# EIDOSLAB/ProgressiveCodec

Measured on AMD Instinct MI355X. Metric: megapixels/s encode+decode (256x256 batches), higher is better.
Workload: dtype f32

## Files before the change

### include/pcodec.h

```cpp
#ifndef PCODEC_H
#define PCODEC_H

#include <stddef.h>
#include <stdint.h>

#ifdef __cplusplus
extern "C" {
#endif

#if defined(__GNUC__)
#define PC_API __attribute__((visibility("default")))
#else
#define PC_API
#endif

enum {
    PC_OK = 0,
    PC_ERR_ARG = -1,
    PC_ERR_INDEX = -2,
    PC_ERR_BUFFER = -3,
    PC_ERR_TRUNCATED = -4,
    PC_ERR_CDF = -5,
    PC_ERR_HIP = -6,
    PC_ERR_NOMEM = -7,
// ... 137 lines not shown
PC_API int pc_codec_profile_begin(pc_codec* c);
PC_API int pc_codec_profile_end(pc_codec* c, int64_t* n_launches, double* total_ms, double* total_flops);
PC_API int pc_codec_profile_bytes(const pc_codec* c, double* total_algorithmic_bytes);
PC_API int pc_profile_set_epoch(int device);
PC_API int pc_codec_profile_intervals(const pc_codec* c, double* t0_ms, double* t1_ms, double* flops, size_t cap, size_t* n);
PC_API int pc_codec_host_stats(const pc_codec* c, double* out, int n);

PC_API int pc_selftest_packed_gelu(uint64_t* n_mismatch, uint64_t* n_nan_payload);

#define PC_TEST_MAX_SEG 8
typedef struct pc_test_conv_desc {
    int nseg;
    const float* seg_ptr[PC_TEST_MAX_SEG];
    int seg_ld[PC_TEST_MAX_SEG];
    int seg_nch[PC_TEST_MAX_SEG];
    int smallc;
    int64_t in_sb, in_sy, in_sx, in_sc;
    int Cin, B, H, W;
    int kind, k, stride;
    int square;
    const float* w; const float* bias; int Cout;
    int epi;
    const float* aux0; int ld0;
    const float* aux1; int ld1;
    const float* fg_gamma; const float* fg_beta;
    float* out;
    int64_t out_sb, out_sy, out_sx, out_sc;
    int pixel_shuffle;
    float* out_relu;
    int ngroup;
    const float* g1_seg0; const float* g1_w; const float* g1_bias; float* g1_out;
    int tile_cfg;
} pc_test_conv_desc;
#define PC_PLAN_UNI_16_3 1
#define PC_PLAN_UNI_32_2 2
#define PC_PLAN_UNI_32_3 3
#define PC_PLAN_UNI_32_2_SQ 4
#define PC_PLAN_UNI_OTHER 5
#define PC_PLAN_L0_64x64 6
#define PC_PLAN_L0_64x64_SMALLC 7
#define PC_PLAN_L0_128x32 8
#define PC_PLAN_L0_128x32_SMALLC 9
#define PC_PLAN_L0_128x128 10
#define PC_PLAN_L0_128x128_SMALLC 11
#define PC_PLAN_IN_GDN 12
#define PC_FORM_SLOW 1
#define PC_FORM_DIRECT 2
#define PC_FORM_TABLE 3
#define PC_FORM_NCHW_PS 4
#define PC_FORM_L0_DIRECT 5
#define PC_FORM_L0_GENERIC 6
#define PC_FORM_IN_GDN 7
PC_API int pc_test_conv(const pc_test_conv_desc* d, int* plan, void* stream);

typedef struct pc_test_stage_desc {
    int size;
    int kind;
    int B;
    int HW;
    int C;
    int H;
    int W;
    const float* scale;
    int ld_scale;
    const float* mu;
    int ld_mu;
    const float* y;
    int ld_y;
    const float* ybase;
    int ld_ybase;
    const float* yadd;
    int ld_yadd;
    const float* thr;
    int mask_mode;
    const float* mask_src;
    int64_t mask_sb;
    const float* table;
    int ntable;
    float bound;
    int32_t* sym;
    int32_t* idx;
    uint8_t* idx8;
    float* mask;
    float* yhat;
    int ld_yhat;
    float* lik;
    int64_t lik_sb;
    const float* x;
    int ld_x;
    const float* aux0;
    const float* aux1;
    float* out;
    float* out2;
    int heads;
    int ws;
    int shift;
    int bias_ji;
    float fscale;
    int inverse;
    float q;
    uint32_t* work;
    int64_t sb;
    const float* thr_bar;
    int mode_star;
    int mode_bar;
} pc_test_stage_desc;
// ... 25 lines not shown
```

### progressivecodec_amd/_lib.py

```python
import ctypes as C
import os

_HERE = os.path.dirname(os.path.abspath(__file__))
LIB_PATH = os.environ.get("PC_LIB") or os.path.join(_HERE, "libpcodec.so")

PC_OK = 0
ERRORS = {-1: "PC_ERR_ARG", -2: "PC_ERR_INDEX", -3: "PC_ERR_BUFFER", -4: "PC_ERR_TRUNCATED", -5: "PC_ERR_CDF",
          -6: "PC_ERR_HIP", -7: "PC_ERR_NOMEM", -8: "PC_ERR_STATE", -9: "PC_ERR_MISSING"}

EXPORTS = [
    "pc_version", "pc_strerror", "pc_last_hip_error", "pc_rans_bound", "pc_rans_encode_with_indexes",
    "pc_rans_decode_with_indexes", "pc_rans_encode_batch", "pc_rans_decode_batch", "pc_pmf_to_quantized_cdf",
    "pc_pack_conv_weight", "pc_conv2d_nhwc", "pc_gdn_nhwc", "pc_win_attention_nhwc", "pc_mask_quantile_threshold",
    "pc_gc_prep_encode", "pc_gc_prep_decode_index", "pc_gc_dequantize", "pc_codec_create", "pc_codec_destroy",
    "pc_codec_set_tensor", "pc_codec_set_tables", "pc_codec_finalize", "pc_codec_set_threads", "pc_codec_compress",
    "pc_codec_num_slices", "pc_codec_get_string", "pc_codec_decompress", "pc_codec_read_tap", "pc_codec_read_tap_i32",
    "pc_codec_profile_begin", "pc_codec_profile_end", "pc_codec_compress_levels", "pc_codec_get_level_string",
    "pc_codec_decompress_levels", "pc_codec_forward", "pc_codec_set_cust_map", "pc_codec_strings_size", "pc_codec_copy_strings",
    "pc_codec_decompress_packed", "pc_host_pool_plan", "pc_rans_decode_stream", "pc_codec_set_scale_table", "pc_codec_profile_bytes", "pc_contract_id", "pc_rans_decode_batch_u8", "pc_codec_set_rem",
    "pc_codec_host_stats", "pc_codec_set_rem_checkpoint", "pc_codec_set_option", "pc_selftest_packed_gelu", "pc_profile_set_epoch", "pc_codec_profile_intervals",
    "pc_codec_set_post_filter", "pc_codec_post_filter",
    "pc_codec_set_model", "pc_codec_wacnn_compress", "pc_codec_wacnn_decompress", "pc_codec_wacnn_forward",
    "pc_test_conv", "pc_codec_set_topology", "pc_test_stage",
]


class PcodecError(RuntimeError):
    def __init__(self, code, where=""):
        self.code = code
        msg = lib().pc_strerror(code).decode() if _lib is not None else ""
        hip = lib().pc_last_hip_error() if (_lib is not None and code == -6) else 0
        super().__init__(f"{where}: {ERRORS.get(code, code)} ({msg})" + (f" hipError={hip}" if hip else ""))


_lib = None


def lib():
    global _lib
    if _lib is None:
        if not os.path.exists(LIB_PATH):
            raise ImportError(
                f"{LIB_PATH} not found: build it with `python -c 'import __graft_entry__ as g; g.build()'` "
                "(hipcc --offload-arch=gfx950).  progressivecodec_amd has no CPU fallback.")
        L = C.CDLL(LIB_PATH)
        vp, i32p, f32p, u8p, sz = C.c_void_p, C.POINTER(C.c_int32), C.POINTER(C.c_float), C.POINTER(C.c_uint8), C.c_size_t
        L.pc_version.restype = C.c_char_p
        L.pc_contract_id.restype = C.c_uint32
        L.pc_strerror.restype = C.c_char_p
        L.pc_strerror.argtypes = [C.c_int]
        L.pc_rans_bound.restype = sz
        L.pc_rans_bound.argtypes = [sz]
        L.pc_rans_encode_with_indexes.argtypes = [vp, vp, sz, vp, C.c_int, C.c_int, vp, vp, vp, sz, C.POINTER(sz)]
        L.pc_rans_decode_with_indexes.argtypes = [vp, sz, vp, sz, vp, C.c_int, C.c_int, vp, vp, vp]
        L.pc_rans_decode_batch_u8.argtypes = [vp, vp, sz, vp, sz, vp, C.c_int, C.c_int, vp, vp, vp, C.c_int]
        L.pc_rans_decode_stream.argtypes = [vp, sz, vp, vp, sz, vp, C.c_int, C.c_int, vp, vp, vp]
        L.pc_host_pool_plan.argtypes = [C.POINTER(C.c_int), C.POINTER(C.c_int), C.POINTER(C.c_int)]
        L.pc_rans_encode_batch.argtypes = [vp, vp, sz, sz, vp, C.c_int, C.c_int, vp, vp, vp, sz, vp, C.c_int]
        L.pc_rans_decode_batch.argtypes = [vp, vp, sz, vp, sz, vp, C.c_int, C.c_int, vp, vp, vp, C.c_int]
        L.pc_pmf_to_quantized_cdf.argtypes = [vp, C.c_int, C.c_int, vp]
        L.pc_pack_conv_weight.argtypes = [vp, C.c_int, C.c_int, C.c_int, C.c_int, vp]
        L.pc_conv2d_nhwc.argtypes = [vp, C.c_int, C.c_int, C.c_int, C.c_int, vp, vp, C.c_int, C.c_int, C.c_int, C.c_int,
                                     C.c_int, C.c_int, vp, vp]
        L.pc_gdn_nhwc.argtypes = [vp, C.c_int, C.c_int, C.c_int, C.c_int, vp, vp, C.c_int, vp, vp]
        L.pc_win_attention_nhwc.argtypes = [vp, vp, C.c_int, C.c_int, C.c_int, C.c_int, C.c_int, C.c_int, C.c_int, vp, vp]
        L.pc_mask_quantile_threshold.argtypes = [vp, C.c_int, C.c_int, C.c_int, C.c_int, C.c_float, vp, vp]
        L.pc_gc_prep_encode.argtypes = [vp, C.c_int, vp, C.c_int, vp, C.c_int, vp, C.c_int, vp, C.c_int, C.c_int, C.c_int,
                                        vp, C.c_int, C.c_float, vp, vp, vp, vp, C.c_int, vp]
        L.pc_gc_prep_decode_index.argtypes = [vp, C.c_int, vp, C.c_int, C.c_int, C.c_int, vp, C.c_int, C.c_float, vp, vp, vp]
        L.pc_gc_dequantize.argtypes = [vp, vp, C.c_int, C.c_int, C.c_int, vp, C.c_int, vp]
        L.pc_codec_create.argtypes = [C.POINTER(vp), C.c_int]
        L.pc_codec_destroy.argtypes = [vp]
        L.pc_codec_destroy.restype = None
        L.pc_codec_set_tensor.argtypes = [vp, C.c_char_p, vp, C.c_int, C.POINTER(C.c_int64), C.c_int]
        L.pc_codec_set_tables.argtypes = [vp, C.c_int, vp, C.c_int, C.c_int, vp, vp]
        L.pc_codec_finalize.argtypes = [vp]
        L.pc_codec_set_threads.argtypes = [vp, C.c_int]
        L.pc_codec_set_option.argtypes = [vp, C.c_char_p, C.c_int]
        if hasattr(L, "pc_selftest_packed_gelu"):
            L.pc_selftest_packed_gelu.argtypes = [C.POINTER(C.c_uint64), C.POINTER(C.c_uint64)]
        if hasattr(L, "pc_test_conv"):
            L.pc_test_conv.argtypes = [vp, C.POINTER(C.c_int), vp]
        if hasattr(L, "pc_test_stage"):
            L.pc_test_stage.argtypes = [vp, C.POINTER(C.c_int), vp]
        L.pc_codec_compress.argtypes = [vp, vp, C.c_int, C.c_int, C.c_int, C.c_double, C.c_int, vp, vp]
        L.pc_codec_num_slices.argtypes = [vp]
        L.pc_codec_get_string.argtypes = [vp, C.c_int, C.c_int, C.POINTER(vp), C.POINTER(sz)]
        L.pc_codec_decompress.argtypes = [vp, vp, vp, C.c_int, vp, vp, C.c_int, C.c_int, C.c_int, C.c_double, C.c_int, vp, vp]
        L.pc_codec_compress_levels.argtypes = [vp, vp, C.c_int, C.c_int, C.c_int, vp, C.c_int, C.c_int, vp, vp]
        L.pc_codec_get_level_string.argtypes = [vp, C.c_int, C.c_int, C.c_int, C.POINTER(vp), C.POINTER(sz)]
        L.pc_codec_decompress_levels.argtypes = [vp, vp, vp, vp, vp, C.c_int, C.c_int, C.c_int, vp, C.c_int, C.c_int, vp, vp]
        L.pc_codec_set_cust_map.argtypes = [vp, vp]
        L.pc_codec_set_rem.argtypes = [vp, vp, C.c_int]
        L.pc_codec_set_rem_checkpoint.argtypes = [vp, vp]
        L.pc_codec_set_post_filter.argtypes = [vp, C.c_int]
        L.pc_codec_post_filter.argtypes = [vp, C.c_int, vp, C.c_int, C.c_int, C.c_int, vp, vp]
        L.pc_codec_set_model.argtypes = [vp, C.c_int]
        L.pc_codec_set_topology.argtypes = [vp, vp]
        L.pc_codec_wacnn_compress.argtypes = [vp, vp, C.c_int, C.c_int, C.c_int, vp]
        L.pc_codec_wacnn_decompress.argtypes = [vp, vp, sz, vp, vp, C.c_int, C.c_int, C.c_int, vp, vp]
        L.pc_codec_wacnn_forward.argtypes = [vp, vp, C.c_int, C.c_int, C.c_int, vp, vp, vp, vp]
        L.pc_codec_strings_size.argtypes = [vp, C.POINTER(sz), C.POINTER(C.c_int)]
        L.pc_codec_copy_strings.argtypes = [vp, vp, sz, vp, sz]
        L.pc_codec_decompress_packed.argtypes = [vp, vp, vp, C.c_int, C.c_int, C.c_int, vp, C.c_int, C.c_int, vp, vp]
        L.pc_codec_forward.argtypes = [vp, vp, C.c_int, C.c_int, C.c_int, C.c_double, C.c_int, vp, vp, vp, vp, C.c_int, vp]
        L.pc_codec_set_scale_table.argtypes = [vp, vp, C.c_int]
        L.pc_codec_read_tap.argtypes = [vp, C.c_char_p, vp, sz, C.POINTER(sz)]
        L.pc_codec_read_tap_i32.argtypes = [vp, C.c_char_p, vp, sz, C.POINTER(sz)]
        L.pc_codec_profile_begin.argtypes = [vp]
        L.pc_profile_set_epoch.argtypes = [C.c_int]
        L.pc_codec_profile_intervals.argtypes = [vp, vp, vp, vp, sz, C.POINTER(sz)]
        L.pc_codec_profile_bytes.argtypes = [vp, C.POINTER(C.c_double)]
        L.pc_codec_host_stats.argtypes = [vp, C.POINTER(C.c_double), C.c_int]
        L.pc_codec_profile_end.argtypes = [vp, C.POINTER(C.c_int64), C.POINTER(C.c_double), C.POINTER(C.c_double)]
        _lib = L
    return _lib


def check(code, where=""):
    if code != PC_OK:
        raise PcodecError(code, where)
```

### progressivecodec_amd/csrc/pc_codec.hip

```cpp
#include <hip/hip_runtime.h>

#include <algorithm>
#include <atomic>
#include <chrono>
#include <condition_variable>
#include <new>
#include <cmath>
#include <cstdio>
#include <cstdlib>
#include <cstring>
#include <functional>
#include <map>
#include <mutex>
#include <thread>
#include <string>
#include <vector>

#include "../../include/pcodec.h"
#include "pc_device.h"
#include "pc_host.h"

static std::atomic<int> g_last_hip{0};
struct pc_codec;
static thread_local pc_codec* g_prof = nullptr;
// ... 44 lines not shown
    bool staging_pending = false;
    pc_rowtab_cache* rowtabs = nullptr;
    std::map<std::string, HostTensor> sd;
    std::vector<void*> weight_allocs;
    std::map<std::string, DevBuf> bufs;
    struct GaW { ConvW c0, c2, c5, c7; GdnW g1, g3, g6; WamW w4, w8; };
    GaW ga[2];
    std::vector<LrrW> rem;
    int rem_levels_loaded = 0;
    int rem_n = 0;
    double rem_check[3] = {0, 0, 0};
    bool multi_enc = false;
    GsW gs[2];
    int post_mode = 0;
    UnetW unet[2];
    ConvW ha[5];
    HsW hms[2], hss[2];
    pc_topology topo{};
    ConvW joiner[NS0][3];
    Stack5W cc_mean[NS0], cc_scale[NS0], lrp[NS0], cc_mean_p[NS0], cc_scale_p[NS0], lrp_p[NS0];
    float* medians = nullptr;
    const float* cust_map = nullptr;
    const float* rem_ckpt = nullptr;
    int opt_serial = 0, opt_lanes_enc = 0, opt_lanes_dec = 0;
    int rem_mu_std = 0;
    float* eb_net = nullptr;
    float* scale_table = nullptr;
    int n_table = 0;
    float scale_bound = 0.11f;
    Tables gc, eb;
    int32_t* h_sym = nullptr; int32_t* h_idx = nullptr; size_t h_cap = 0;
    int res_slices = 0, res_B = 0;
    std::vector<char> res_level_coded;
    std::vector<hipEvent_t> lvl_events;
    hipStream_t pipe_stream = nullptr;
    std::vector<hipEvent_t> pipe_ev;
    std::vector<std::vector<uint8_t>> y_strings;
    std::vector<std::vector<uint8_t>> z_strings;
    int n_threads = 0;
    bool profile = false;
    bool profile_in_schedule = false;
    bool serial_profile() const { return profile && !profile_in_schedule; }
    std::mutex prof_mu;
    std::vector<hipEvent_t> ev;
    size_t ev_used = 0;
    double prof_flops = 0.0, prof_bytes = 0.0;
    struct ProfRec { int M, N, K, nphase, epi; double flops, bytes; double t0_ms, t1_ms; };
    std::vector<ProfRec> prof_rec;
    struct Lane { hipStream_t sA = nullptr; hipEvent_t eDone = nullptr; };
    std::vector<Lane> lanes;
    hipEvent_t eFork = nullptr;
    std::mutex buf_mu;
    double t_host_decode_ms = 0.0;
    double t_compress_ms = 0.0, t_host_encode_ms = 0.0, t_host_encode_exposed_ms = 0.0, t_decompress_ms = 0.0;
    double n_sym_encoded = 0.0, n_sym_decoded = 0.0;
    int last_B = 0, last_h16 = 0, last_w16 = 0;

    template <typename T> int buf(const std::string& name, size_t count, T** out)
    {
        std::lock_guard<std::mutex> lk(buf_mu);
        DevBuf& d = bufs[name];
        const size_t need = count * sizeof(T);
        if (d.bytes < need) {
            if (d.p) (void)hipFree(d.p);
            d.p = nullptr; d.bytes = 0;
            HIPCHK(hipMalloc(&d.p, need));
            d.bytes = need;
        }
        *out = reinterpret_cast<T*>(d.p);
        return PC_OK;
    }
};

namespace {

struct LaunchState {
    pc_codec* prof0;
    pc_rowtab_cache* rowtabs0;
    explicit LaunchState(pc_codec* c) : prof0(g_prof), rowtabs0(g_rowtabs) { g_prof = c && c->profile ? c : nullptr; g_rowtabs = c ? c->rowtabs : nullptr; }
    ~LaunchState() { g_prof = prof0; g_rowtabs = rowtabs0; }
    LaunchState(const LaunchState&) = delete;
    LaunchState& operator=(const LaunchState&) = delete;
};

double now_ms() { return std::chrono::duration<double, std::milli>(std::chrono::steady_clock::now().time_since_epoch()).count(); }

int launch_conv(const pc_conv_params& q_in, hipStream_t st, int* plan = nullptr)
{
    pc_conv_params q = q_in;
    q.rowtab_cache = g_rowtabs;
    pc_codec* c = g_prof;
    if (!c) return pc_conv_launch(q, st, plan);
    long taps = 0;
    for (int ph = 0; ph < q.nphase; ++ph) taps += q.ntap[ph];
    const double ng = q.ngroup == 2 ? 2.0 : 1.0;
    double fl = 2.0 * (double)q.M * (double)q.Cout * (double)taps * (double)q.Cin * ng;
    if (q.fg_gamma) fl += 2.0 * (double)q.M * (double)q.Cout * (double)q.Cout;
    double by = 0.0;
    for (int sg = 0; sg < q.nseg; ++sg) by += 4.0 * (double)q.B * q.H * q.W * q.seg[sg].nch * (sg == 0 ? ng : 1.0);
    by += ng * 4.0 * ((double)taps * q.Cin * q.Cout + q.Cout);
    if (q.fg_gamma) by += 4.0 * ((double)q.Cout * q.Cout + q.Cout);
    by += ng * 4.0 * (double)q.nphase * q.M * q.Cout;
    if (q.aux0 && q.epi != PC_EPI_NONE && q.epi != PC_EPI_GELU && q.epi != PC_EPI_CLAMP01) by += 4.0 * (double)q.nphase * q.M * q.Cout;
    if (q.aux1 && (q.epi == PC_EPI_GATE || q.epi == PC_EPI_LRP_ADD)) by += 4.0 * (double)q.nphase * q.M * q.Cout;
    hipEvent_t e0, e1;
    {
        std::lock_guard<std::mutex> lk(c->prof_mu);
        if (c->ev_used + 2 > c->ev.size()) {
            const size_t old = c->ev.size();
            c->ev.resize(old + 512);
            for (size_t i = old; i < c->ev.size(); ++i) HIPCHK(hipEventCreate(&c->ev[i]));
        }
        c->prof_flops += fl;
        c->prof_bytes += by;
        c->prof_rec.push_back({q.M, q.Cout, (int)(taps * q.Cin / q.nphase), q.nphase, q.epi, fl, by, 0.0, 0.0});
        e0 = c->ev[c->ev_used++]; e1 = c->ev[c->ev_used++];
    }
    HIPCHK(hipEventRecord(e0, st));
    const int r = pc_conv_launch(q, st, plan);
    HIPCHK(hipEventRecord(e1, st));
    return r;
}

const HostTensor* find(const pc_codec* c, const std::string& k, int dtype, std::initializer_list<int64_t> shape)
{
    auto it = c->sd.find(k);
    if (it == c->sd.end() || it->second.dtype != dtype) return nullptr;
    if (it->second.shape.size() != shape.size()) return nullptr;
    size_t i = 0;
    for (int64_t s : shape) if (it->second.shape[i++] != s) return nullptr;
    return &it->second;
}

int upload(pc_codec* c, const std::vector<float>& h, float** dev)
{
    void* p = nullptr;
    HIPCHK(hipMalloc(&p, std::max<size_t>(h.size(), 4) * sizeof(float)));
    HIPCHK(hipMemcpy(p, h.data(), h.size() * sizeof(float), hipMemcpyHostToDevice));
    c->weight_allocs.push_back(p);
    *dev = reinterpret_cast<float*>(p);
    return PC_OK;
}

int load_conv(pc_codec* c, const std::string& p, int Cin, int Cout, int k, int kind, ConvW* out)
{
    const HostTensor* w = kind == 0 ? find(c, p + ".weight", PC_F32, {Cout, Cin, k, k}) : find(c, p + ".weight", PC_F32, {Cin, Cout, k, k});
    const HostTensor* b = find(c, p + ".bias", PC_F32, {Cout});
    if (!w || !b) { std::fprintf(stderr, "[pcodec] missing/mis-shaped tensor %s\n", p.c_str()); return PC_ERR_MISSING; }
    std::vector<float> packed((size_t)k * k * Cin * Cout);
    PCCHK(pc_pack_conv_weight(reinterpret_cast<const float*>(w->data.data()), kind, Cout, Cin, k, packed.data()));
    PCCHK(upload(c, packed, &out->w));
    std::vector<float> bias(reinterpret_cast<const float*>(b->data.data()), reinterpret_cast<const float*>(b->data.data()) + Cout);
    PCCHK(upload(c, bias, &out->b));
    out->Cin = Cin; out->Cout = Cout; out->k = k; out->kind = kind; out->layout = pc_conv_weight_layout(kind, Cin, Cout, k);
    return PC_OK;
}

// ... 188 lines not shown
                for (int kx = px; kx < 5; kx += 2) {
                    q.dy[ph][t] = ((py + 2 - ky) / 2); q.dx[ph][t] = ((px + 2 - kx) / 2);
                    q.wtap[ph][t] = ky * 5 + kx;
                    ++t;
                }
            q.ntap[ph] = t; q.ooy[ph] = py; q.oox[ph] = px;
        }
}

int conv_geometry(pc_conv_params& q, int kind, int k, int stride, int H, int W, int B, bool pixel_shuffle)
{
    if (B <= 0 || H <= 0 || W <= 0) return PC_ERR_ARG;
    q.B = B; q.H = H; q.W = W;
    q.Ho = H; q.Wo = W;
    if (kind == 0) {
        if (k <= 0 || k > 5 || stride <= 0) return PC_ERR_ARG;
        fill_conv_taps(q, k, stride);
        q.Ho = (H + 2 * (k / 2) - k) / stride + 1;
        q.Wo = (W + 2 * (k / 2) - k) / stride + 1;
    } else if (kind == 1) fill_deconv_taps(q);
    else if (kind == 2) fill_subpixel_taps(q);
    else return PC_ERR_ARG;
    q.outH = q.osy * q.Ho; q.outW = q.osx * q.Wo;
    q.M = B * q.Ho * q.Wo;
    q.pixel_shuffle = (pixel_shuffle || kind == 2) ? 1 : 0;
    if (q.pixel_shuffle) { q.outH *= 2; q.outW *= 2; }
    return PC_OK;
}

struct Group1 { const ConvW* w; const float* seg0; float* out; };

int conv_n(hipStream_t st, const ConvW& w, const Seg* segs, int nseg, int B, int H, int W, int stride,
           float* out, int ldo, int epi, const float* aux0 = nullptr, int ld0 = 0, const float* aux1 = nullptr, int ld1 = 0,
           bool pixel_shuffle = false, const Group1* g1 = nullptr, float* out_relu = nullptr)
{
    pc_conv_params q;
    std::memset(&q, 0, sizeof(q));
    int cin = 0;
    for (int j = 0; j < nseg; ++j) {
        const Seg& s = segs[j];
        if (s.nch == 0) continue;
        if (q.nseg >= PC_MAX_SEG) return PC_ERR_ARG;
        q.seg[q.nseg].ptr = s.p; q.seg[q.nseg].ld = s.ld; q.seg[q.nseg].nch = s.nch; ++q.nseg; cin += s.nch;
    }
    if (cin != w.Cin) return PC_ERR_ARG;
    q.Cin = cin;
    q.w = w.w; q.wlayout = w.layout; q.bias = w.b; q.Cout = w.Cout;
    q.epi = epi; q.aux0 = aux0; q.ld0 = ld0; q.aux1 = aux1; q.ld1 = ld1;
    q.out = out; q.out_relu = out_relu;
    PCCHK(conv_geometry(q, w.kind == 0 ? 0 : 1, w.k, stride, H, W, B, pixel_shuffle));
    q.out_sc = 1; q.out_sx = ldo; q.out_sy = (int64_t)q.outW * ldo; q.out_sb = (int64_t)q.outH * q.outW * ldo;
    if (g1) {
        if (g1->w->Cin != w.Cin || g1->w->Cout != w.Cout || g1->w->k != w.k || g1->w->layout != 1 || w.layout != 1) return PC_ERR_ARG;
        q.ngroup = 2; q.g1_seg0 = g1->seg0; q.g1_w = g1->w->w; q.g1_bias = g1->w->b; q.g1_out = g1->out;
    }
    return launch_conv(q, st);
}

int conv(hipStream_t st, const ConvW& w, std::initializer_list<Seg> segs, int B, int H, int W, int stride,
         float* out, int ldo, int epi, const float* aux0 = nullptr, int ld0 = 0, const float* aux1 = nullptr, int ld1 = 0,
         bool pixel_shuffle = false, const Group1* g1 = nullptr, float* out_relu = nullptr)
{
    return conv_n(st, w, segs.begin(), (int)segs.size(), B, H, W, stride, out, ldo, epi, aux0, ld0, aux1, ld1, pixel_shuffle, g1, out_relu);
}

int gdn(hipStream_t st, const GdnW& g, const float* x, int B, int H, int W, bool inverse, float* out, int* plan = nullptr)
{
    pc_conv_params q;
    std::memset(&q, 0, sizeof(q));
    q.nseg = 1; q.seg[0].ptr = x; q.seg[0].ld = g.C; q.seg[0].nch = g.C; q.Cin = g.C;
    q.B = B; q.H = H; q.W = W; q.square = 1;
    fill_conv_taps(q, 1, 1);
    q.w = g.gamma; q.wlayout = 1; q.bias = g.beta; q.Cout = g.C;
    q.Ho = H; q.Wo = W; q.outH = H; q.outW = W; q.M = B * H * W;
    q.out = out; q.out_sc = 1; q.out_sx = g.C; q.out_sy = (int64_t)W * g.C; q.out_sb = (int64_t)H * W * g.C;
    q.epi = inverse ? PC_EPI_IGDN : PC_EPI_GDN; q.aux0 = x; q.ld0 = g.C;
    return launch_conv(q, st, plan);
}

int ru(hipStream_t st, const RuW& r, const float* x, int C, int B, int H, int W, float* t1, float* t2, float* out)
{
    PCCHK(conv(st, r.c0, {{x, C, C}}, B, H, W, 1, t1, C / 2, PC_EPI_GELU));
    PCCHK(conv(st, r.c2, {{t1, C / 2, C / 2}}, B, H, W, 1, t2, C / 2, PC_EPI_GELU));
    PCCHK(conv(st, r.c4, {{t2, C / 2, C / 2}}, B, H, W, 1, out, C, PC_EPI_RES_GELU, x, C));
    return PC_OK;
}

int wam(pc_codec* c, hipStream_t st, const WamW& w, const float* x, int B, int H, int W, float* out, int ldo = 0)
{
    const int C = w.C;
    if (ldo == 0) ldo = C;
    const size_t M = (size_t)B * H * W;
    float *t1, *t2, *a0, *a1, *qkv, *o;
    PCCHK(c->buf("wam_t1", M * (C / 2), &t1));
    PCCHK(c->buf("wam_t2", M * (C / 2), &t2));
    PCCHK(c->buf("wam_a0", M * C, &a0));
    PCCHK(c->buf("wam_a1", M * C, &a1));
    PCCHK(c->buf("wam_b0", M * C, &o));
    PCCHK(c->buf("wam_qkv", M * 3 * C, &qkv));
    float* b1;
    PCCHK(c->buf("wam_b1", M * C, &b1));
    PCCHK(ru(st, w.a[0], x, C, B, H, W, t1, t2, a0));
    PCCHK(ru(st, w.a[1], a0, C, B, H, W, t1, t2, a1));
    PCCHK(ru(st, w.a[2], a1, C, B, H, W, t1, t2, a0));
    PCCHK(conv(st, w.qkv, {{x, C, C}}, B, H, W, 1, qkv, 3 * C, PC_EPI_NONE));
    PCCHK(pc_win_attention_launch(qkv, w.bias, B, H, W, C, HEADS, w.ws, w.shift, (float)std::pow((double)(C / HEADS), -0.5), a1, st, 1));
    PCCHK(conv(st, w.proj, {{a1, C, C}}, B, H, W, 1, o, C, PC_EPI_RES, x, C));
// ... 4 lines not shown
    return PC_OK;
}

int stack5_n(pc_codec* c, hipStream_t st, const Stack5W& s, const Seg* segs, int nseg, int B, int h, int w, float* out, int ldo, int epi,
             const char* tag, const float* aux0 = nullptr, int ld0 = 0, const float* aux1 = nullptr, int ld1 = 0)
{
    const size_t M = (size_t)B * h * w;
    float *t0, *t1;
    PCCHK(c->buf(std::string(tag) + "_t0", M * 224, &t0));
    PCCHK(c->buf(std::string(tag) + "_t1", M * 176, &t1));
    PCCHK(conv_n(st, s.c[0], segs, nseg, B, h, w, 1, t0, 224, PC_EPI_GELU));
    PCCHK(conv(st, s.c[1], {{t0, 224, 224}}, B, h, w, 1, t1, 176, PC_EPI_GELU));
    PCCHK(conv(st, s.c[2], {{t1, 176, 176}}, B, h, w, 1, t0, 128, PC_EPI_GELU));
    PCCHK(conv(st, s.c[3], {{t0, 128, 128}}, B, h, w, 1, t1, 64, PC_EPI_GELU));
    PCCHK(conv(st, s.c[4], {{t1, 64, 64}}, B, h, w, 1, out, ldo, epi, aux0, ld0, aux1, ld1));
    return PC_OK;
}

int stack5(pc_codec* c, hipStream_t st, const Stack5W& s, std::initializer_list<Seg> segs, int B, int h, int w,
           float* out, int ldo, int epi, const float* aux0 = nullptr, int ld0 = 0, const float* aux1 = nullptr, int ld1 = 0,
           const char* tag = "s5")
{
    return stack5_n(c, st, s, segs.begin(), (int)segs.size(), B, h, w, out, ldo, epi, tag, aux0, ld0, aux1, ld1);
}

int stack5_pair_n(pc_codec* c, hipStream_t st, const Stack5W& sm, const Stack5W& ss, const Seg* segs_mean, int nseg,
                  const float* seg0_scale, int B, int h, int w, float* out_mean, float* out_scale, const char* tagm, const char* tags)
{
    const size_t M = (size_t)B * h * w;
    float *m0, *m1, *s0, *s1;
    PCCHK(c->buf(std::string(tagm) + "_t0", M * 224, &m0));
    PCCHK(c->buf(std::string(tagm) + "_t1", M * 176, &m1));
    PCCHK(c->buf(std::string(tags) + "_t0", M * 224, &s0));
    PCCHK(c->buf(std::string(tags) + "_t1", M * 176, &s1));
    Group1 g{&ss.c[0], seg0_scale, s0};
    PCCHK(conv_n(st, sm.c[0], segs_mean, nseg, B, h, w, 1, m0, 224, PC_EPI_GELU, nullptr, 0, nullptr, 0, false, &g));
    g = Group1{&ss.c[1], s0, s1};
    PCCHK(conv(st, sm.c[1], {{m0, 224, 224}}, B, h, w, 1, m1, 176, PC_EPI_GELU, nullptr, 0, nullptr, 0, false, &g));
    g = Group1{&ss.c[2], s1, s0};
    PCCHK(conv(st, sm.c[2], {{m1, 176, 176}}, B, h, w, 1, m0, 128, PC_EPI_GELU, nullptr, 0, nullptr, 0, false, &g));
    g = Group1{&ss.c[3], s0, s1};
    PCCHK(conv(st, sm.c[3], {{m0, 128, 128}}, B, h, w, 1, m1, 64, PC_EPI_GELU, nullptr, 0, nullptr, 0, false, &g));
    g = Group1{&ss.c[4], s1, out_scale};
    PCCHK(conv(st, sm.c[4], {{m1, 64, 64}}, B, h, w, 1, out_mean, SLICE, PC_EPI_NONE, nullptr, 0, nullptr, 0, false, &g));
    return PC_OK;
}

int stack5_pair(pc_codec* c, hipStream_t st, const Stack5W& sm, const Stack5W& ss, std::initializer_list<Seg> segs_mean,
                const float* seg0_scale, int B, int h, int w, float* out_mean, float* out_scale, const char* tagm, const char* tags)
{
    return stack5_pair_n(c, st, sm, ss, segs_mean.begin(), (int)segs_mean.size(), seg0_scale, B, h, w, out_mean, out_scale, tagm, tags);
}

int hs(pc_codec* c, hipStream_t st, const HsW& h, const float* z, int B, int zh, int zw, float* out, int ldo)
{
    const size_t M = (size_t)B * zh * zw;
    float *t0, *t1, *t2, *t3;
    PCCHK(c->buf("hs_t0", M * 192, &t0));
    PCCHK(c->buf("hs_t1", M * 4 * 224, &t1));
    PCCHK(c->buf("hs_t2", M * 4 * 256, &t2));
    PCCHK(c->buf("hs_t3", M * 16 * 288, &t3));
    PCCHK(conv(st, h.c0, {{z, 192, 192}}, B, zh, zw, 1, t0, 192, PC_EPI_GELU));
    PCCHK(conv(st, h.c2, {{t0, 192, 192}}, B, zh, zw, 1, t1, 224, PC_EPI_GELU, nullptr, 0, nullptr, 0, true));
    PCCHK(conv(st, h.c4, {{t1, 224, 224}}, B, 2 * zh, 2 * zw, 1, t2, 256, PC_EPI_GELU));
    PCCHK(conv(st, h.c6, {{t2, 256, 256}}, B, 2 * zh, 2 * zw, 1, t3, 288, PC_EPI_GELU, nullptr, 0, nullptr, 0, true));
    PCCHK(conv(st, h.c8, {{t3, 288, 288}}, B, 4 * zh, 4 * zw, 1, out, ldo, PC_EPI_NONE));
    return PC_OK;
}

int g_a_net(pc_codec* c, hipStream_t st, const pc_codec::GaW& g, const float* x, int B, int H, int W, float* y, int ldy)
{
    const int Cy = g.c7.Cout;
    float *t0, *t1, *t2, *t3, *t4;
    PCCHK(c->buf("ga_t0", (size_t)B * (H / 2) * (W / 2) * NCH, &t0));
    PCCHK(c->buf("ga_t1", (size_t)B * (H / 2) * (W / 2) * NCH, &t1));
    PCCHK(c->buf("ga_t2", (size_t)B * (H / 4) * (W / 4) * NCH, &t2));
    PCCHK(c->buf("ga_t3", (size_t)B * (H / 4) * (W / 4) * NCH, &t3));
    PCCHK(c->buf("ga_t4", (size_t)B * (H / 16) * (W / 16) * MLAT, &t4));
    {
        pc_conv_params q;
        std::memset(&q, 0, sizeof(q));
        q.nseg = 1; q.seg[0].ptr = x; q.seg[0].ld = 0; q.seg[0].nch = 3; q.Cin = 3; q.smallc = 1;
        q.B = B; q.H = H; q.W = W;
        q.in_sb = (int64_t)3 * H * W; q.in_sc = (int64_t)H * W; q.in_sy = W; q.in_sx = 1;
        fill_conv_taps(q, 5, 2);
        q.w = g.c0.w; q.bias = g.c0.b; q.Cout = NCH;
        q.Ho = H / 2; q.Wo = W / 2; q.outH = q.Ho; q.outW = q.Wo; q.M = B * q.Ho * q.Wo;
        q.fg_gamma = g.g1.gamma; q.fg_beta = g.g1.beta;
        q.out = t1; q.out_sc = 1; q.out_sx = NCH; q.out_sy = (int64_t)q.Wo * NCH; q.out_sb = (int64_t)q.Ho * q.Wo * NCH;
        PCCHK(launch_conv(q, st));
    }
    PCCHK(conv(st, g.c2, {{t1, NCH, NCH}}, B, H / 2, W / 2, 2, t2, NCH, PC_EPI_NONE));
    PCCHK(gdn(st, g.g3, t2, B, H / 4, W / 4, false, t3));
    PCCHK(wam(c, st, g.w4, t3, B, H / 4, W / 4, t2));
    PCCHK(conv(st, g.c5, {{t2, NCH, NCH}}, B, H / 4, W / 4, 2, t0, NCH, PC_EPI_NONE));
    PCCHK(gdn(st, g.g6, t0, B, H / 8, W / 8, false, t1));
    PCCHK(conv(st, g.c7, {{t1, NCH, NCH}}, B, H / 8, W / 8, 2, t4, Cy, PC_EPI_NONE));
    PCCHK(wam(c, st, g.w8, t4, B, H / 16, W / 16, y, ldy));
    return PC_OK;
}

int g_a(pc_codec* c, hipStream_t st, const float* x, int B, int H, int W, float* y)
{
    if (!c->multi_enc) return g_a_net(c, st, c->ga[0], x, B, H, W, y, MLAT);
    PCCHK(g_a_net(c, st, c->ga[0], x, B, H, W, y, MLAT));
    return g_a_net(c, st, c->ga[1], x, B, H, W, y + D0, MLAT);
// ... 200 lines not shown
            for (int kx = 0; kx < k; ++kx)
                for (int ci = 0; ci < Cin; ++ci) {
                    float* dst = out + (((size_t)(ky * k + kx) * Cin) + ci) * Cout;
                    for (int co = 0; co < Cout; ++co) dst[co] = src(co, ci, ky, kx);
                }
    } else {
        for (int ky = 0; ky < k; ++ky)
            for (int kx = 0; kx < k; ++kx)
                for (int co = 0; co < Cout; ++co) {
                    float* dst = out + (((size_t)(ky * k + kx) * Cout) + co) * Cin;
                    for (int ci = 0; ci < Cin; ++ci) dst[ci] = src(co, ci, ky, kx);
                }
    }
    return PC_OK;
}

extern "C" int pc_conv2d_nhwc(const float* x, int B, int H, int W, int Cin, const float* w_packed, const float* bias,
                              int kind, int Cout, int k, int stride, int act, int tile_cfg, float* out, void* stream)
{
    if (!x || !w_packed || !out) return PC_ERR_ARG;
    pc_conv_params q;
    std::memset(&q, 0, sizeof(q));
    q.nseg = 1; q.seg[0].ptr = x; q.seg[0].ld = Cin; q.seg[0].nch = Cin; q.Cin = Cin;
    if (Cin % 16) { q.smallc = 1; q.in_sc = 1; q.in_sx = Cin; q.in_sy = (int64_t)W * Cin; q.in_sb = (int64_t)H * W * Cin; if (kind != 0) return PC_ERR_ARG; }
    q.w = w_packed; q.bias = bias; q.Cout = Cout; q.epi = act ? PC_EPI_GELU : PC_EPI_NONE; q.tile_cfg = tile_cfg;
    q.wlayout = pc_conv_weight_layout(kind, Cin, Cout, k);
    if (kind != 0 && k != 5) return PC_ERR_ARG;
    PCCHK(conv_geometry(q, kind == 0 ? 0 : 1, k, stride, H, W, B, false));
    q.out = out; q.out_sc = 1; q.out_sx = Cout; q.out_sy = (int64_t)q.outW * Cout; q.out_sb = (int64_t)q.outH * q.outW * Cout;
    return pc_conv_launch(q, (hipStream_t)stream);
}

extern "C" int pc_test_conv(const pc_test_conv_desc* d, int* plan, void* stream)
{
    if (plan) plan[0] = plan[1] = 0;
    if (!d || !d->out || !d->w || d->nseg < 1 || d->nseg > PC_MAX_SEG || d->B <= 0 || d->H <= 0 || d->W <= 0) return PC_ERR_ARG;
    pc_conv_params q;
    std::memset(&q, 0, sizeof(q));
    q.nseg = d->nseg;
    for (int s = 0; s < d->nseg; ++s) { q.seg[s].ptr = d->seg_ptr[s]; q.seg[s].ld = d->seg_ld[s]; q.seg[s].nch = d->seg_nch[s]; }
    q.smallc = d->smallc ? 1 : 0;
    q.in_sb = d->in_sb; q.in_sy = d->in_sy; q.in_sx = d->in_sx; q.in_sc = d->in_sc;
    q.Cin = d->Cin;
    q.square = d->square ? 1 : 0;
    q.w = d->w; q.bias = d->bias; q.Cout = d->Cout; q.tile_cfg = d->tile_cfg;
    q.epi = d->epi; q.aux0 = d->aux0; q.ld0 = d->ld0; q.aux1 = d->aux1; q.ld1 = d->ld1;
    q.fg_gamma = d->fg_gamma; q.fg_beta = d->fg_beta;
    if (d->kind == 2 && d->Cout != 12) return PC_ERR_ARG;
    PCCHK(conv_geometry(q, d->kind, d->k, d->stride, d->H, d->W, d->B, d->pixel_shuffle != 0));
    if (d->kind == 0) q.wlayout = q.square ? 1 : pc_conv_weight_layout(0, d->Cin, d->Cout, d->k);
    else q.wlayout = d->kind == 1 ? pc_conv_weight_layout(1, d->Cin, d->Cout, 5) : 1;
    q.out = d->out; q.out_sb = d->out_sb; q.out_sy = d->out_sy; q.out_sx = d->out_sx; q.out_sc = d->out_sc;
    q.out_relu = d->out_relu;
    if (d->ngroup == 2) { q.ngroup = 2; q.g1_seg0 = d->g1_seg0; q.g1_w = d->g1_w; q.g1_bias = d->g1_bias; q.g1_out = d->g1_out; }
    return pc_conv_launch(q, (hipStream_t)stream, plan);
}

extern "C" int pc_test_stage(const pc_test_stage_desc* d, int* plan, void* stream)
{
    if (plan) plan[0] = 0;
    if (!d || d->size != (int)sizeof(pc_test_stage_desc)) return PC_ERR_ARG;
    hipStream_t st = (hipStream_t)stream;
    int chosen = 0, rc = PC_ERR_ARG;
    switch (d->kind) {
    case PC_STAGE_PREP_ENC: case PC_STAGE_PREP_DEC_INDEX: case PC_STAGE_PREP_DEQUANT: {
        pc_prep_params p;
        std::memset(&p, 0, sizeof(p));
        p.B = d->B; p.HW = d->HW; p.C = d->C;
        p.scale = d->scale; p.ld_scale = d->ld_scale; p.mu = d->mu; p.ld_mu = d->ld_mu; p.y = d->y; p.ld_y = d->ld_y;
        p.ybase = d->ybase; p.ld_ybase = d->ld_ybase; p.yadd = d->yadd; p.ld_yadd = d->ld_yadd;
        p.thr = d->thr; p.mask_mode = d->mask_mode; p.mask_src = d->mask_src; p.mask_sb = d->mask_sb;
        p.table = d->table; p.ntable = d->ntable; p.bound = d->bound;
        p.sym = d->sym; p.idx = d->idx; p.idx8 = d->idx8; p.mask = d->mask; p.yhat = d->yhat; p.ld_yhat = d->ld_yhat;
        p.lik = d->lik; p.lik_sb = d->lik_sb;
        if (d->kind == PC_STAGE_PREP_ENC) {
            if (!p.scale || !p.mu || !p.y || !p.sym || !p.idx || !p.yhat || !p.table || (p.mask_mode == 1 && !p.thr)) return PC_ERR_ARG;
            rc = pc_prep_enc_launch(p, st, &chosen);
        } else if (d->kind == PC_STAGE_PREP_DEC_INDEX) {
            if (!p.scale || !p.idx || !p.table || (p.mask_mode == 1 && !p.thr)) return PC_ERR_ARG;
            rc = pc_prep_dec_index_launch(p, st, &chosen);
        } else {
            if (!p.sym || !p.mu || !p.yhat) return PC_ERR_ARG;
            rc = pc_prep_dec_dequant_launch(p, st, &chosen);
        }
        break;
    }
    case PC_STAGE_ATTENTION:
        rc = pc_win_attention_launch(d->x, d->aux0, d->B, d->H, d->W, d->C, d->heads, d->ws, d->shift, d->fscale, d->out, st, d->bias_ji, &chosen);
        break;
    case PC_STAGE_GDN: {
        if (!d->x || !d->aux0 || !d->aux1 || !d->out || d->C <= 0 || d->C % 16 || d->B <= 0 || d->H <= 0 || d->W <= 0) return PC_ERR_ARG;
        GdnW g; g.beta = const_cast<float*>(d->aux0); g.gamma = const_cast<float*>(d->aux1); g.C = d->C;
        int cp[2] = {0, 0};
        rc = gdn(st, g, d->x, d->B, d->H, d->W, d->inverse != 0, d->out, cp);
        chosen = PC_SPLAN_GDN + cp[0];
        break;
    }
    case PC_STAGE_QUANTILE:
        if (!d->scale || !d->out) return PC_ERR_ARG;
        rc = pc_quantile_thr_launch(d->scale, d->ld_scale, d->B, d->HW, d->C, d->q, d->out, d->work, st, d->sb, &chosen);
        break;
    case PC_STAGE_EB_QUANT:
        rc = pc_eb_quant_launch(d->x, d->B, d->HW, d->C, d->aux0, d->sym, d->out, st); chosen = PC_SPLAN_SINGLE; break;
    case PC_STAGE_EB_DEQUANT:
        rc = pc_eb_dequant_launch(d->sym, d->B, d->HW, d->C, d->aux0, d->out, st); chosen = PC_SPLAN_SINGLE; break;
    case PC_STAGE_EB_LIK:
        rc = pc_eb_likelihood_launch(d->sym, d->B, d->HW, d->C, d->aux0, d->aux1, d->out, st); chosen = PC_SPLAN_SINGLE; break;
// ... 608 lines not shown
        PCCHK(rem_rb(st, L.base_rep[j], {{x, ldx, SLICE}}, x, ldx, B, h, w, t1, ts, o));
        x = o; ldx = SLICE;
    }
    PCCHK(rem_rb(st, L.ent_base[0], {{mu_b, SLICE, SLICE}, {sd_b, SLICE, SLICE}}, nullptr, 0, B, h, w, t1, ts, L.n_sub == 1 ? fb : pa));
    x = pa; ldx = SLICE;
    for (int j = 1; j < L.n_sub; ++j) {
        float* o = j == L.n_sub - 1 ? fb : (j & 1 ? pb : pa);
        PCCHK(rem_rb(st, L.ent_base[j], {{x, ldx, SLICE}}, x, ldx, B, h, w, t1, ts, o));
        x = o;
    }
    PCCHK(rem_rb(st, L.enc[0], {{fl, SLICE, SLICE}, {fb, SLICE, SLICE}, {fp, SLICE, SLICE}}, nullptr, 0, B, h, w, t1, ts, pa));
    x = pa;
    for (int j = 1; j < L.n_enc; ++j) {
        float* o = (j & 1) ? pb : pa;
        const int ci = L.enc[j].c1.Cin;
        PCCHK(rem_rb(st, L.enc[j], {{x, ci, ci}}, x, ci, B, h, w, t1, ts, o));
        x = o;
    }
    if (c->rem_mu_std) return pc_rem_combine_launch(x, 2 * SLICE, sc_i, SLICE, nb, k.HW, thr2, mode_star, thr2 + k.B, mode_bar, st, mu_i, SLICE);
    return pc_rem_combine_launch(x, SLICE, sc_i, SLICE, nb, k.HW, thr2, mode_star, thr2 + k.B, mode_bar, st);
}

int support_count(const pc_codec* c, int i) { return std::min(5 - c->topo.support_deficit, i); }

void support_segs(const ChainCtx& k, int i, int b0, bool std, Seg* sg, int* n)
{
    const pc_topology& T = k.c->topo;
    auto mu_tot = [&](int j) { return k.mut ? k.mut + slice_off(k, j, b0) : k.mu + slice_off(k, NS0 + j, b0); };
    auto sc = [&](int j) { return k.scale + slice_off(k, NS0 + j, b0); };
    const int s = support_count(k.c, i);
    for (int e = i - s; e < i; ++e) {
        const float* p;
        if (!std) p = mu_tot(e);
        else if (!k.lik) p = T.support_std ? sc(e) : mu_tot(e);
        else p = (e & 1) ? sc(e >> 1) : (T.support_std ? sc(e >> 1) : mu_tot(e >> 1));
        sg[(*n)++] = {p, SLICE, SLICE};
    }
}

int joiner(const ChainCtx& k, int i, int b0, int nb, const float* enhanced, hipStream_t st, const std::string& tag)
{
    pc_codec* c = k.c;
    const size_t pi = (size_t)k.HW, m = (size_t)nb * pi;
    float *ja, *jb;
    PCCHK(c->buf("jn_a" + tag, m * 64, &ja));
    PCCHK(c->buf("jn_b" + tag, m * 64, &jb));
    const float* yb = img(k.yb, b0, pi * D0) + 32 * i;
    float* ye = img(k.ye, b0, pi * D0) + 32 * i;
    PCCHK(conv(st, c->joiner[i][0], {{enhanced, SLICE, SLICE}, {yb, D0, SLICE}}, nb, k.h, k.w, 1, ja, 64, PC_EPI_GELU));
    PCCHK(conv(st, c->joiner[i][1], {{ja, 64, 64}}, nb, k.h, k.w, 1, jb, 64, PC_EPI_GELU));
    return conv(st, c->joiner[i][2], {{jb, 64, 64}}, nb, k.h, k.w, 1, ye, D0, PC_EPI_NONE);
}

int chain_workspace(pc_codec* c, const std::string& tag, size_t m)
{
    float* d;
    for (const char* base : {"s5m", "s5s"}) {
        PCCHK(c->buf(base + tag + "_t0", m * 224, &d));
        PCCHK(c->buf(base + tag + "_t1", m * 176, &d));
    }
    if (!c->topo.joiner_cond) return PC_OK;
    PCCHK(c->buf("jn_pm" + tag, m * SLICE, &d));
    PCCHK(c->buf("jn_a" + tag, m * 64, &d));
    return c->buf("jn_b" + tag, m * 64, &d);
}

int chain_params(const ChainCtx& k, int step, int b0, int nb, hipStream_t st, const std::string& tag)
{
    pc_codec* c = k.c;
    const size_t pi = (size_t)k.HW;
    float* lm = img(k.lm, b0, pi * MLAT); float* ls = img(k.ls, b0, pi * MLAT);
    float* yb = img(k.yb, b0, pi * D0); float* ye = img(k.ye, b0, pi * D0);
    float* mu_i = k.mu + slice_off(k, step, b0);
    float* sc_i = k.scale + slice_off(k, step, b0);
    const std::string tm = "s5m" + tag, ts = "s5s" + tag;
    if (step < NS0) {
        const int i = step, ns = std::min(5, i);
        return stack5_pair(c, st, c->cc_mean[i], c->cc_scale[i], {{lm, MLAT, D0}, {yb, D0, 32 * ns}}, ls, nb, k.h, k.w, mu_i, sc_i, tm.c_str(), ts.c_str());
    }
    const int i = step - NS0;
    const pc_topology& T = c->topo;
    if (!T.all_scalable) {
        const int s = support_count(c, i);
        PCCHK(stack5_pair(c, st, c->cc_mean_p[i], c->cc_scale_p[i], {{lm + D0, MLAT, D0}, {yb + 32 * i, D0, 32}, {ye + 32 * (i - s), D0, 32 * s}},
                          ls + D0, nb, k.h, k.w, mu_i, sc_i, tm.c_str(), ts.c_str()));
    } else {
        Seg sm[PC_MAX_SEG], ss[PC_MAX_SEG];
        int nm = 0, ns = 0;
        sm[nm++] = {lm + D0, MLAT, D0}; sm[nm++] = {yb + 32 * i, D0, 32};
        ss[ns++] = {ls + D0, MLAT, D0}; ss[ns++] = {yb + 32 * i, D0, 32};
        support_segs(k, i, b0, false, sm, &nm);
        support_segs(k, i, b0, true, ss, &ns);
        bool same = nm == ns;
        for (int j = 2; same && j < nm; ++j) same = sm[j].p == ss[j].p;
        if (same) {
            PCCHK(stack5_pair_n(c, st, c->cc_mean_p[i], c->cc_scale_p[i], sm, nm, ls + D0, nb, k.h, k.w, mu_i, sc_i, tm.c_str(), ts.c_str()));
        } else {
            PCCHK(stack5_n(c, st, c->cc_mean_p[i], sm, nm, nb, k.h, k.w, mu_i, SLICE, PC_EPI_NONE, tm.c_str()));
            PCCHK(stack5_n(c, st, c->cc_scale_p[i], ss, ns, nb, k.h, k.w, sc_i, SLICE, PC_EPI_NONE, ts.c_str()));
        }
    }
    if (k.mut) {
        float* t1;
        PCCHK(c->buf(tm + "_t1", (size_t)nb * pi * 176, &t1));
        PCCHK(conv(st, c->cc_mean_p[i].c[4], {{t1, 64, 64}}, nb, k.h, k.w, 1, k.mut + slice_off(k, i, b0), SLICE,
                   PC_EPI_RES, yb + 32 * i, D0));
    }
    PCCHK(rem_refine(k, i, b0, nb, mu_i, sc_i, st, tag));
    if (k.mode == 1) PCCHK(mask_threshold(k, i, b0, nb, sc_i, st, tag));
    return PC_OK;
}

int chain_lrp(const ChainCtx& k, int step, int b0, int nb, hipStream_t sA, const std::string& tag)
{
    pc_codec* c = k.c;
    const size_t pi = (size_t)k.HW;
    float* lm = img(k.lm, b0, pi * MLAT);
    float* yb = img(k.yb, b0, pi * D0); float* ye = img(k.ye, b0, pi * D0);
    const std::string tm = "s5m" + tag;
    if (step < NS0) {
        const int i = step;
        if (i < 5)
            return stack5(c, sA, c->lrp[i], {{lm, MLAT, D0}, {yb, D0, 32 * (i + 1)}}, nb, k.h, k.w, yb + 32 * i, D0, PC_EPI_LRP, yb + 32 * i, D0, nullptr, 0, tm.c_str());
        return stack5(c, sA, c->lrp[i], {{lm, MLAT, D0}, {yb, D0, 160}, {yb + 32 * i, D0, 32}}, nb, k.h, k.w, yb + 32 * i, D0, PC_EPI_LRP, yb + 32 * i, D0, nullptr, 0, tm.c_str());
    }
    const int i = step - NS0;
    const pc_topology& T = c->topo;
    const bool rbl = T.residual_before_lrp && k.lik;
    if (!T.all_scalable && !T.joiner_cond && !rbl) {
        const int s = support_count(c, i);
        return stack5(c, sA, c->lrp_p[i], {{lm + D0, MLAT, D0}, {yb + 32 * i, D0, 32}, {ye + 32 * (i - s), D0, 32 * (s + 1)}}, nb, k.h, k.w,
                      ye + 32 * i, D0, PC_EPI_LRP_ADD, ye + 32 * i, D0, yb + 32 * i, D0, tm.c_str());
    }
    Seg sg[PC_MAX_SEG];
    int n = 0;
    sg[n++] = {lm + D0, MLAT, D0}; sg[n++] = {yb + 32 * i, D0, 32};
    if (T.all_scalable) support_segs(k, i, b0, false, sg, &n);
    else { const int s = support_count(c, i); if (s) sg[n++] = {ye + 32 * (i - s), D0, 32 * s}; }
    sg[n++] = {ye + 32 * i, D0, 32};
    if (rbl || !T.joiner_cond) {
        return stack5_n(c, sA, c->lrp_p[i], sg, n, nb, k.h, k.w, ye + 32 * i, D0, rbl ? PC_EPI_LRP : PC_EPI_LRP_ADD, tm.c_str(), ye + 32 * i, D0,
                        rbl ? nullptr : yb + 32 * i, D0);
    }
    float* pm;
    PCCHK(c->buf("jn_pm" + tag, (size_t)nb * pi * SLICE, &pm));
    PCCHK(stack5_n(c, sA, c->lrp_p[i], sg, n, nb, k.h, k.w, pm, SLICE, PC_EPI_LRP, tm.c_str(), ye + 32 * i, D0));
    return joiner(k, i, b0, nb, pm, sA, tag);
}

int encode_lane(const ChainCtx& k, int b0, int nb, hipStream_t sA, const std::string& tag)
{
    pc_codec* c = k.c;
    const size_t pi = (size_t)k.HW;
    for (int step = k.step0; step < k.step1; ++step) {
        PCCHK(chain_wait(k, step, sA));
        PCCHK(chain_params(k, step, b0, nb, sA, tag));
        const size_t so = slice_off(k, step, b0);
        pc_prep_params p = chain_prep(k, step, b0, nb);
        p.mu = k.mu + so; p.ld_mu = SLICE; p.y = img(k.y, b0, pi * MLAT) + 32 * step; p.ld_y = MLAT;
        p.sym = k.sym + so;
        p.lik = k.lik ? k.lik + ((size_t)b0 * k.lik_nch + (size_t)32 * step) * pi : nullptr;
        p.lik_sb = (int64_t)k.lik_nch * (int64_t)pi;
        if (step < NS0) {
            p.yhat = img(k.yb, b0, pi * D0) + 32 * step; p.ld_yhat = D0;
            PCCHK(pc_prep_enc_launch(p, sA));
        } else {
            const int i = step - NS0;
            const pc_topology& T = c->topo;
            p.mask = k.masks ? k.masks + slice_off(k, i, b0) : nullptr;
            const bool rbl = T.residual_before_lrp && k.lik;
            p.yhat = img(k.ye, b0, pi * D0) + 32 * i; p.ld_yhat = D0;
            if (rbl && T.joiner_cond) { PCCHK(c->buf("jn_pm" + tag, (size_t)nb * pi * SLICE, &p.yhat)); p.ld_yhat = SLICE; }
            if (rbl && !T.joiner_cond) p.yadd = img(k.yb, b0, pi * D0) + 32 * i;
            p.ld_yadd = D0;
            if (!T.no_delta_encode) p.ybase = img(k.y, b0, pi * MLAT) + 32 * i;
            p.ld_ybase = MLAT;
            PCCHK(pc_prep_enc_launch(p, sA));
            if (rbl && T.joiner_cond) PCCHK(joiner(k, i, b0, nb, p.yhat, sA, tag));
        }
        PCCHK(chain_lrp(k, step, b0, nb, sA, tag));
        PCCHK(chain_signal(k, step, sA));
    }
    return PC_OK;
}

int decode_lane(const ChainCtx& k, int b0, int nb, hipStream_t sA, const std::string& tag, const uint8_t* const* y_strings, const size_t* y_lens,
                int nt)
{
    pc_codec* c = k.c;
    HIPCHK(hipSetDevice(c->device));
    LaunchState launch(c);
    const size_t pi = (size_t)k.HW, per = (size_t)SLICE * k.HW;
    int32_t* h_idx = c->h_idx + k.h_off + (size_t)b0 * per;
    int32_t* h_sym = c->h_sym + k.h_off + (size_t)b0 * per;
    for (int step = k.step0; step < k.step1; ++step) {
        PCCHK(chain_wait(k, step, sA));
        PCCHK(chain_params(k, step, b0, nb, sA, tag));
        const size_t so = slice_off(k, step, b0);
        const bool e = step >= NS0;
        const int i = e ? step - NS0 : step;
        pc_prep_params p = chain_prep(k, step, b0, nb);
        p.idx8 = k.idx8 + so;
        PCCHK(pc_prep_dec_index_launch(p, sA));
        uint8_t* h_idx8 = reinterpret_cast<uint8_t*>(h_idx);
        HIPCHK(hipMemcpyAsync(h_idx8, k.idx8 + so, per * nb, hipMemcpyDeviceToHost, sA));
        HIPCHK(hipStreamSynchronize(sA));
        const double td0 = now_ms();
        const size_t slot = e ? (size_t)NS0 + (size_t)NS0 * k.level + i : (size_t)step;
        PCCHK(pc::rans_decode_u8_batch(y_strings + slot * k.B + b0, y_lens + slot * k.B + b0, nb, h_idx8, per, c->gc.dec(), h_sym, nt));
        { std::lock_guard<std::mutex> lk(c->buf_mu); c->t_host_decode_ms += now_ms() - td0; }
        HIPCHK(hipMemcpyAsync(k.sym + so, h_sym, per * nb * 4, hipMemcpyHostToDevice, sA));
        float* dst = e ? img(k.ye, b0, pi * D0) + 32 * i : img(k.yb, b0, pi * D0) + 32 * i;
        PCCHK(pc_gc_dequantize(k.sym + so, k.mu + so, SLICE, nb, k.HW, dst, D0, sA));
        PCCHK(chain_lrp(k, step, b0, nb, sA, tag));
        PCCHK(chain_signal(k, step, sA));
    }
    return PC_OK;
}

int run_chain(const ChainCtx& k, hipStream_t st, bool decode, const uint8_t* const* y_strings, const size_t* y_lens)
{
    pc_codec* c = k.c;
    if (c->serial_profile() || c->opt_serial)
        return decode ? decode_lane(k, 0, k.B, st, "", y_strings, y_lens, c->n_threads == 1 ? 1 : 0)
                      : encode_lane(k, 0, k.B, st, "");
    const int nl = lane_count(c, k.B, decode);
    PCCHK(ensure_lanes(c, nl));
    for (int g = 0; g < nl; ++g) {
        const int b0 = (int)((long)k.B * g / nl), nb = (int)((long)k.B * (g + 1) / nl) - b0;
        PCCHK(chain_workspace(c, std::to_string(g), (size_t)nb * k.HW));
    }
    HIPCHK(hipEventRecord(c->eFork, st));
    for (int g = 0; g < nl; ++g) HIPCHK(hipStreamWaitEvent(c->lanes[g].sA, c->eFork, 0));
    std::vector<int> rcs(nl, PC_OK);
    std::vector<std::thread> threads;
    for (int g = 0; g < nl; ++g) {
        const int b0 = (int)((long)k.B * g / nl), nb = (int)((long)k.B * (g + 1) / nl) - b0;
        const hipStream_t sA = c->lanes[g].sA;
        const std::string tag = std::to_string(g);
        if (decode)
            threads.emplace_back([&, g, b0, nb, sA, tag] { rcs[g] = decode_lane(k, b0, nb, sA, tag, y_strings, y_lens, c->n_threads == 1 ? 1 : 0); });
        else
            rcs[g] = encode_lane(k, b0, nb, sA, tag);
    }
    for (auto& t : threads) t.join();
    int rc = PC_OK;
    for (int g = 0; g < nl; ++g) {
        pc_codec::Lane& L = c->lanes[g];
        hipError_t e = hipEventRecord(L.eDone, L.sA);
        if (e == hipSuccess) e = hipStreamWaitEvent(st, L.eDone, 0);
        if (e != hipSuccess && rc == PC_OK) { g_last_hip = (int)e; rc = PC_ERR_HIP; }
    }
    for (int g = 0; g < nl; ++g) if (rcs[g] != PC_OK) return rcs[g];
    return rc;
}

}

namespace {

int encode_streams(pc_codec* c, const int32_t* hs, const int32_t* hi, int first_slot, int n_slots, int B, size_t per,
                   const int32_t* z_sym, const int32_t* z_idx, size_t per_z)
{
    std::atomic<int> rc{PC_OK};
    const size_t n_y_jobs = (size_t)n_slots * B;
    auto job = [&](size_t j) {
        const bool is_z = j >= n_y_jobs;
        const size_t n = is_z ? per_z : per;
        const int32_t* sym = is_z ? z_sym + (j - n_y_jobs) * per_z : hs + j * per;
        const int32_t* idx = is_z ? z_idx + (j - n_y_jobs) * per_z : hi + j * per;
        const Tables& t = is_z ? c->eb : c->gc;
        std::vector<uint8_t>& dst = is_z ? c->z_strings[j - n_y_jobs] : c->y_strings[(size_t)first_slot * B + j];
        dst.resize(pc_rans_bound(n));
        size_t len = 0;
        const int r = pc_rans_encode_with_indexes(sym, idx, n, t.cdf.data(), t.n, t.stride, t.len.data(), t.off.data(), dst.data(),
                                                  dst.size(), &len);
        if (r != PC_OK) rc = r;
        dst.resize(len);
    };
    const size_t n_jobs = n_y_jobs + (z_sym ? (size_t)B : 0);
    if (c->n_threads == 1) for (size_t j = 0; j < n_jobs; ++j) job(j);
    else pc::default_pool().parallel_for(n_jobs, job);
    return rc;
}

bool pipeline_enabled(const pc_codec* c)
{
    return !c->serial_profile() && !c->opt_serial;
}

int second_level_set(pc_codec* c, const ChainCtx& k, bool decoder, ChainCtx* k2)
{
    *k2 = k;
    PCCHK(c->buf("yhat_enh_L2", k.M * D0, &k2->ye));
    PCCHK(c->buf("mu_L2", k.M * SLICE * 2 * NS0, &k2->mu));
    PCCHK(c->buf("scale_L2", k.M * SLICE * 2 * NS0, &k2->scale));
    if (k.mut) PCCHK(c->buf("mut_L2", k.M * SLICE * NS0, &k2->mut));
    PCCHK(c->buf("thr_L2", (size_t)k.B * NS0, &k2->thr));
    PCCHK(c->buf("sym_L2", k.M * SLICE * 2 * NS0, &k2->sym));
    PCCHK(c->buf("idx_L2", k.M * SLICE * 2 * NS0, &k2->idx));
    if (decoder) PCCHK(c->buf("idx8_L2", k.M * SLICE * 2 * NS0, &k2->idx8));
    return PC_OK;
}

int ensure_pipeline(pc_codec* c, size_t M)
{
    if (!c->pipe_stream) {
        HIPCHK(hipStreamCreateWithFlags(&c->pipe_stream, hipStreamNonBlocking));
        c->pipe_ev.resize(NS0 + 2);
        for (auto& e : c->pipe_ev) HIPCHK(hipEventCreateWithFlags(&e, hipEventDisableTiming));
    }
    for (const char* tag : {"PA", "PB"}) PCCHK(chain_workspace(c, tag, M));
    return PC_OK;
}

int pipe_fork(pc_codec* c, hipStream_t st)
{
    HIPCHK(hipEventRecord(c->pipe_ev[NS0], st));
    HIPCHK(hipStreamWaitEvent(c->pipe_stream, c->pipe_ev[NS0], 0));
    return PC_OK;
}

int pipe_join(pc_codec* c, hipStream_t st)
{
    HIPCHK(hipEventRecord(c->pipe_ev[NS0 + 1], c->pipe_stream));
    HIPCHK(hipStreamWaitEvent(st, c->pipe_ev[NS0 + 1], 0));
    return PC_OK;
}

enum class CallKind { compress, forward, decompress };

int call_setup(pc_codec* c, CallKind kind, int B, int a, int b, ChainCtx* k)
{
    std::memset(k, 0, sizeof(*k));
    const int zh = kind == CallKind::decompress ? a : a / 64, zw = kind == CallKind::decompress ? b : b / 64;
    const int h = 4 * zh, w = 4 * zw;
    const size_t M = (size_t)B * h * w, MZ = (size_t)B * zh * zw * NCH;
    c->last_B = B; c->last_h16 = h; c->last_w16 = w;
    if (kind != CallKind::decompress) PCCHK(c->buf("y", M * MLAT, &k->y));
    PCCHK(c->buf("latent_means", M * MLAT, &k->lm));
    PCCHK(c->buf("latent_scales", M * MLAT, &k->ls));
    PCCHK(c->buf("yhat_base", M * D0, &k->yb));
    PCCHK(c->buf("yhat_enh", M * D0, &k->ye));
    PCCHK(c->buf("mu", M * SLICE * 2 * NS0, &k->mu));
    PCCHK(c->buf("scale", M * SLICE * 2 * NS0, &k->scale));
    if (c->topo.total_mu_rep && c->topo.all_scalable) PCCHK(c->buf("mut", M * SLICE * NS0, &k->mut));
    PCCHK(c->buf("thr", (size_t)B * NS0, &k->thr));
    PCCHK(c->buf("sym", M * SLICE * 2 * NS0, &k->sym));
    PCCHK(c->buf("idx", M * SLICE * 2 * NS0, &k->idx));
    if (kind == CallKind::decompress) PCCHK(c->buf("idx8", M * SLICE * 2 * NS0, &k->idx8));
    if (kind != CallKind::decompress) PCCHK(c->buf("z", MZ, &k->z));
    PCCHK(c->buf("z_hat", MZ, &k->z_hat));
    PCCHK(c->buf("z_sym", MZ, &k->z_sym));
    k->c = c; k->B = B; k->h = h; k->w = w; k->HW = h * w; k->M = M;
    k->zh = zh; k->zw = zw; k->ZHW = zh * zw;
    k->step0 = 0; k->step1 = NS0;
    k->mu_base = k->mu; k->scale_base = k->scale;
    if (kind != CallKind::forward) {
        k->cust_map = c->cust_map; c->cust_map = nullptr;
        k->rem_ckpt = c->rem_ckpt; c->rem_ckpt = nullptr;
    }
    return PC_OK;
}

ChainCtx level_ctx(const ChainCtx& base, int level, double quality, int mask_pol)
// ... 46 lines not shown
}

struct BusyGuard {
    pc_codec* c;
    bool ok;
    explicit BusyGuard(pc_codec* cc) : c(cc), ok(false) { bool f = false; ok = c->busy.compare_exchange_strong(f, true, std::memory_order_acquire); }
    ~BusyGuard() { if (ok) c->busy.store(false, std::memory_order_release); }
};
struct CallOrder {
    pc_codec* c;
    hipStream_t st;
    bool on;
    int rc;
    CallOrder(pc_codec* cc, hipStream_t s, bool go) : c(cc), st(s), on(go), rc(PC_OK)
    {
        if (!on) return;
        if (!c->call_done) { if (hipEventCreateWithFlags(&c->call_done, hipEventDisableTiming) != hipSuccess) { c->call_done = nullptr; rc = PC_ERR_HIP; } }
        else if (hipStreamWaitEvent(st, c->call_done, 0) != hipSuccess) rc = PC_ERR_HIP;
    }
    ~CallOrder()
    {
        if (!on) return;
        if (c->pipe_stream && c->pipe_ev.size() > (size_t)NS0 + 1) (void)pipe_join(c, st);
        if (c->call_done) (void)hipEventRecord(c->call_done, st);
    }
};
struct CallScope {
    BusyGuard busy;
    int rc;
    CallOrder order;
    LaunchState launch;
    CallScope(pc_codec* c, hipStream_t st) : busy(c), rc(enter(c, busy.ok)), order(c, st, rc == PC_OK), launch(rc == PC_OK ? c : nullptr) { if (rc == PC_OK) rc = order.rc; }
    static int enter(pc_codec* c, bool is_free) { if (!is_free) return PC_ERR_STATE; HIPCHK(hipSetDevice(c->device)); return PC_OK; }
};

void eb_indexes(int32_t* idx, size_t n, int ZHW) { for (size_t e = 0; e < n; ++e) idx[e] = (int32_t)((e / ZHW) % NCH); }

int encoder_front(const ChainCtx& k, hipStream_t st, const float* x, bool enh, float* z_lik)
{
    pc_codec* c = k.c;
    PCCHK(g_a(c, st, x, k.B, 16 * k.h, 16 * k.w, k.y));
    PCCHK(h_a(c, st, k.y, k.B, k.h, k.w, k.z));
    PCCHK(pc_eb_quant_launch(k.z, k.B, k.ZHW, NCH, c->medians, k.z_sym, k.z_hat, st));
    if (z_lik) PCCHK(pc_eb_likelihood_launch(k.z_sym, k.B, k.ZHW, NCH, c->medians, c->eb_net, z_lik, st));
    return hyper(c, st, k.z_hat, k.B, k.zh, k.zw, enh ? 1.0 : 0.0, k.lm, k.ls);
}

int decoder_front(const ChainCtx& k, hipStream_t st, const uint8_t* const* z_strings, const size_t* z_lens, bool enh)
{
    pc_codec* c = k.c;
    const size_t per = (size_t)SLICE * k.HW, per_z = (size_t)NCH * k.ZHW;
    if (c->staging_pending) { HIPCHK(hipEventSynchronize(c->staging_done)); c->staging_pending = false; }
    if (!c->staging_done) HIPCHK(hipEventCreateWithFlags(&c->staging_done, hipEventDisableTiming));
    PCCHK(ensure_host_staging(c, std::max(per * k.B, per_z * k.B)));
    eb_indexes(c->h_idx, per_z * k.B, k.ZHW);
    PCCHK(pc_rans_decode_batch(z_strings, z_lens, k.B, c->h_idx, per_z, c->eb.cdf.data(), c->eb.n, c->eb.stride, c->eb.len.data(),
                               c->eb.off.data(), c->h_sym, c->n_threads == 1 ? 1 : 0));
    HIPCHK(hipMemcpyAsync(k.z_sym, c->h_sym, per_z * k.B * 4, hipMemcpyHostToDevice, st));
    PCCHK(pc_eb_dequant_launch(k.z_sym, k.B, k.ZHW, NCH, c->medians, k.z_hat, st));
    HIPCHK(hipStreamSynchronize(st));
    return hyper(c, st, k.z_hat, k.B, k.zh, k.zw, enh ? 1.0 : 0.0, k.lm, k.ls);
}

int compress_impl(pc_codec* c, const float* x, int B, int H, int W, const double* qualities, int n_levels, int mask_pol,
                  float* const* masks_out, hipStream_t st)
{
    if (!c || !x || !qualities || n_levels < 1 || B <= 0 || H <= 0 || W <= 0 || (H % 64) || (W % 64)) return PC_ERR_ARG;
    if (mask_pol < PC_MASK_POINT_BASED_STD || mask_pol > PC_MASK_THREE_LEVELS_STD) return PC_ERR_ARG;
    if (!c->finalized || !c->gc.ok() || !c->eb.ok() || c->model != PC_MODEL_CHANNEL) return PC_ERR_STATE;
    if (c->eb.n != NCH) return PC_ERR_STATE;
    CallScope call(c, st);
    if (call.rc != PC_OK) return call.rc;
    bool any_enh = false;
    for (int l = 0; l < n_levels; ++l) any_enh = any_enh || !(qualities[l] <= 0);

    ChainCtx k;
    PCCHK(call_setup(c, CallKind::compress, B, H, W, &k));
    const size_t n_half = (size_t)NS0 * k.M * SLICE, n_z = (size_t)B * k.ZHW * NCH;
    const size_t per = (size_t)SLICE * k.HW, per_z = (size_t)NCH * k.ZHW;
    PCCHK(ensure_host_staging(c, 3 * n_half + n_z));
    while ((int)c->lvl_events.size() < n_levels + 1) {
        hipEvent_t e;
        HIPCHK(hipEventCreateWithFlags(&e, hipEventDisableTiming));
        c->lvl_events.push_back(e);
    }
    c->res_slices = NS0 + NS0 * n_levels; c->res_B = B;
    c->res_level_coded.assign(n_levels, 0);
    c->y_strings.assign((size_t)c->res_slices * B, {});
    c->z_strings.assign(B, {});
    static const bool timing = std::getenv("PC_TIMING") != nullptr;
    const double t0 = now_ms();
    double t_host = 0.0, t_enc_last = 0.0;

    PCCHK(encoder_front(k, st, x, any_enh, nullptr));
    int first_coded = -1, n_coded_total = 0;
    for (int l = 0; l < n_levels; ++l) if (!(qualities[l] <= 0)) { ++n_coded_total; if (first_coded < 0) first_coded = l; }
    auto base_d2h = [&]() -> int {
        HIPCHK(hipMemcpyAsync(c->h_sym, k.sym, n_half * 4, hipMemcpyDeviceToHost, st));
        HIPCHK(hipMemcpyAsync(c->h_idx, k.idx, n_half * 4, hipMemcpyDeviceToHost, st));
        HIPCHK(hipMemcpyAsync(c->h_sym + 3 * n_half, k.z_sym, n_z * 4, hipMemcpyDeviceToHost, st));
        HIPCHK(hipEventRecord(c->lvl_events[0], st));
        return PC_OK;
    };
    const bool piped = pipeline_enabled(c) && first_coded >= 0 && lane_count(c, B, false) == 1;
    const bool two_levels = piped && n_coded_total >= 2;
    ChainCtx k2;
    if (two_levels) PCCHK(second_level_set(c, k, false, &k2));
// ... 130 lines not shown
                                float* y_lik, float* z_lik, float* masks_out, int force_enhanced, void* stream)
{
    if (!c || !x || !x_hat || !y_lik || !z_lik || B <= 0 || H <= 0 || W <= 0 || (H % 64) || (W % 64)) return PC_ERR_ARG;
    if (mask_pol < PC_MASK_POINT_BASED_STD || mask_pol > PC_MASK_THREE_LEVELS_STD) return PC_ERR_ARG;
    if (!c->finalized || !c->eb_net || c->model != PC_MODEL_CHANNEL) return PC_ERR_STATE;
    hipStream_t st = (hipStream_t)stream;
    CallScope call(c, st);
    if (call.rc != PC_OK) return call.rc;
    const bool enh = quality != 0 || force_enhanced != 0;

    ChainCtx k;
    PCCHK(call_setup(c, CallKind::forward, B, H, W, &k));
    k.lik = y_lik; k.lik_nch = enh ? 2 * D0 : D0;

    PCCHK(encoder_front(k, st, x, enh, z_lik));
    ChainCtx ke = level_ctx(k, 0, quality, mask_pol);
    ke.masks = masks_out;
    if (enh && pipeline_enabled(c) && lane_count(c, B, false) == 1) {
        PCCHK(encode_pipelined(k, ke, st, true, nullptr));
    } else {
        PCCHK(run_chain(k, st, false, nullptr, nullptr));
        if (enh) PCCHK(run_chain(ke, st, false, nullptr, nullptr));
    }
    PCCHK(synth(c, st, c->gs[enh ? 1 : 0], enh ? k.ye : k.yb, B, k.h, k.w, x_hat));
    return PC_OK;
}

namespace {

int decompress_impl(pc_codec* c, const uint8_t* const* y_strings, const size_t* y_lens, const uint8_t* const* z_strings,
                    const size_t* z_lens, int B, int zh, int zw, const double* qualities, int n_levels, int mask_pol, float* x_hat,
                    hipStream_t st)
{
    if (!c || !y_strings || !y_lens || !z_strings || !z_lens || !x_hat || !qualities || n_levels < 1 || B <= 0 || zh <= 0 || zw <= 0) return PC_ERR_ARG;
    if (mask_pol < PC_MASK_POINT_BASED_STD || mask_pol > PC_MASK_THREE_LEVELS_STD) return PC_ERR_ARG;
    if (!c->finalized || !c->gc.ok() || !c->eb.ok() || c->eb.n != NCH || c->model != PC_MODEL_CHANNEL) return PC_ERR_STATE;
    CallScope call(c, st);
    if (call.rc != PC_OK) return call.rc;
    bool any_enh = false;
    for (int l = 0; l < n_levels; ++l) any_enh = any_enh || qualities[l] != 0;

    ChainCtx k;
    PCCHK(call_setup(c, CallKind::decompress, B, zh, zw, &k));
    const int h = k.h, w = k.w;
    const size_t M = k.M, per = (size_t)SLICE * k.HW, per_z = (size_t)NCH * k.ZHW;
    struct StagingMark {
        pc_codec* c; hipStream_t st; bool marked;
        void mark() { if (c->staging_done && hipEventRecord(c->staging_done, st) == hipSuccess) { c->staging_pending = true; marked = true; } }
        ~StagingMark() { if (!marked) mark(); }
    } staging_mark{c, st, false};
    PCCHK(decoder_front(k, st, z_strings, z_lens, any_enh));
    const int nt = c->n_threads == 1 ? 1 : 0;
    c->t_host_decode_ms = 0.0;
    int first_enh = -1;
    for (int l = 0; l < n_levels && first_enh < 0; ++l) if (qualities[l] != 0) first_enh = l;
    const bool piped = pipeline_enabled(c) && first_enh >= 0;
    if (piped) {
        PCCHK(ensure_pipeline(c, M));
        PCCHK(ensure_host_staging(c, std::max(2 * per * B, per_z * B)));
        SliceSignal recorded;
        ChainCtx kb = k;
        kb.sig = c->pipe_ev.data(); kb.sig_count = &recorded;
        ChainCtx ke = level_ctx(k, first_enh, qualities[first_enh], mask_pol);
        ke.waitv = c->pipe_ev.data(); ke.wait_count = &recorded; ke.h_off = per * B;
        PCCHK(decode_pair(kb, ke, st, y_strings, y_lens, nt));
    } else {
        PCCHK(run_chain(k, st, true, y_strings, y_lens));
    }
    staging_mark.mark();
    const size_t img_elems = (size_t)B * 3 * (16 * h) * (16 * w);
    std::vector<int> rest;
    for (int l = 0; l < n_levels; ++l) if (qualities[l] != 0 && !(piped && l == first_enh)) rest.push_back(l);
    if (piped && !rest.empty()) {
        ChainCtx k2;
        PCCHK(second_level_set(c, k, true, &k2));
        for (int l = 0; l < n_levels; ++l) if (qualities[l] == 0) PCCHK(synth(c, st, c->gs[0], k.yb, B, h, w, x_hat + (size_t)l * img_elems));
        PCCHK(synth(c, st, c->gs[1], k.ye, B, h, w, x_hat + (size_t)first_enh * img_elems));
        for (size_t p = 0; p < rest.size(); p += 2) {
            const int la = rest[p], lb = p + 1 < rest.size() ? rest[p + 1] : -1;
            const ChainCtx ka = level_ctx(k2, la, qualities[la], mask_pol);
            if (lb >= 0) {
                ChainCtx kb = level_ctx(k, lb, qualities[lb], mask_pol);
                kb.h_off = per * B;
                PCCHK(decode_pair(ka, kb, st, y_strings, y_lens, nt));
            } else {
                PCCHK(decode_lane(ka, 0, B, st, "PA", y_strings, y_lens, nt));
            }
            staging_mark.mark();
            PCCHK(synth(c, st, c->gs[1], ka.ye, B, h, w, x_hat + (size_t)la * img_elems));
            if (lb >= 0) PCCHK(synth(c, st, c->gs[1], k.ye, B, h, w, x_hat + (size_t)lb * img_elems));
        }
    } else
    for (int l = 0; l < n_levels; ++l) {
        float* out = x_hat + (size_t)l * img_elems;
        if (qualities[l] == 0) {
            PCCHK(synth(c, st, c->gs[0], k.yb, B, h, w, out));
            continue;
        }
        if (!(piped && l == first_enh)) {
            PCCHK(run_chain(level_ctx(k, l, qualities[l], mask_pol), st, true, y_strings, y_lens));
            staging_mark.mark();
        }
        PCCHK(synth(c, st, c->gs[1], k.ye, B, h, w, out));
    }
    {
        int n_enh = 0;
        for (int l = 0; l < n_levels; ++l) n_enh += qualities[l] != 0 ? 1 : 0;
        c->n_sym_decoded = (double)per_z * B + (double)per * B * NS0 * (1 + n_enh);
    }
    if (std::getenv("PC_TIMING")) std::fprintf(stderr, "[pcodec] decompress: %d level(s), host rANS decode (summed over lanes) %.2f ms\n", n_levels, c->t_host_decode_ms);
    return PC_OK;
}

}

extern "C" int pc_codec_decompress(pc_codec* c, const uint8_t* const* y_strings, const size_t* y_lens, int n_slices,
                                   const uint8_t* const* z_strings, const size_t* z_lens, int B, int zh, int zw,
// ... 114 lines not shown
{
    if (!c || !x || !x_hat || !y_lik || !z_lik || B <= 0 || H <= 0 || W <= 0 || (H % 64) || (W % 64)) return PC_ERR_ARG;
    if (!c->finalized || !c->eb_net || c->model != PC_MODEL_WACNN) return PC_ERR_STATE;
    hipStream_t st = (hipStream_t)stream;
    CallScope call(c, st);
    if (call.rc != PC_OK) return call.rc;
    ChainCtx k;
    PCCHK(call_setup(c, CallKind::forward, B, H, W, &k));
    k.lik = y_lik; k.lik_nch = D0;
    PCCHK(encoder_front(k, st, x, false, z_lik));
    PCCHK(run_chain(k, st, false, nullptr, nullptr));
    return g_s(c, st, c->gs[0], k.yb, B, k.h, k.w, x_hat, PC_EPI_NONE);
}

extern "C" int pc_codec_read_tap(pc_codec* c, const char* name, float* host_out, size_t cap, size_t* n)
{
    if (!c || !name || !n) return PC_ERR_ARG;
    auto it = c->bufs.find(name);
    if (it == c->bufs.end()) return PC_ERR_ARG;
    const size_t cnt = it->second.bytes / 4;
    *n = cnt;
    if (!host_out) return PC_OK;
    const size_t m = std::min(cnt, cap);
    HIPCHK(hipSetDevice(c->device));
    HIPCHK(hipDeviceSynchronize());
    HIPCHK(hipMemcpy(host_out, it->second.p, m * 4, hipMemcpyDeviceToHost));
    return PC_OK;
}

extern "C" int pc_codec_read_tap_i32(pc_codec* c, const char* name, int32_t* host_out, size_t cap, size_t* n)
{
    return pc_codec_read_tap(c, name, reinterpret_cast<float*>(host_out), cap, n);
}

extern "C" int pc_codec_profile_begin(pc_codec* c)
{
    if (!c) return PC_ERR_ARG;
    c->profile = true; c->ev_used = 0; c->prof_flops = 0.0; c->prof_bytes = 0.0; c->prof_rec.clear();
    return PC_OK;
}

extern "C" int pc_codec_profile_bytes(const pc_codec* c, double* total_algorithmic_bytes)
{
    if (!c || !total_algorithmic_bytes) return PC_ERR_ARG;
    *total_algorithmic_bytes = c->prof_bytes;
    return PC_OK;
}

extern "C" int pc_codec_host_stats(const pc_codec* c, double* out, int n)
{
    if (!c || !out || n < 6) return PC_ERR_ARG;
    out[0] = c->t_compress_ms; out[1] = c->t_host_encode_ms; out[2] = c->t_host_encode_exposed_ms;
    out[3] = c->t_host_decode_ms; out[4] = c->n_sym_encoded; out[5] = c->n_sym_decoded;
    return PC_OK;
}

static std::mutex g_epoch_mu;
static hipEvent_t g_epoch[16] = {};
extern "C" int pc_profile_set_epoch(int device)
{
    if (device < 0 || device >= 16) return PC_ERR_ARG;
    HIPCHK(hipSetDevice(device));
    HIPCHK(hipDeviceSynchronize());
    std::lock_guard<std::mutex> lk(g_epoch_mu);
    if (!g_epoch[device]) HIPCHK(hipEventCreate(&g_epoch[device]));
    HIPCHK(hipEventRecord(g_epoch[device], nullptr));
    HIPCHK(hipEventSynchronize(g_epoch[device]));
    return PC_OK;
}

extern "C" int pc_codec_profile_end(pc_codec* c, int64_t* n_launches, double* total_ms, double* total_flops)
{
    if (!c || !n_launches || !total_ms || !total_flops) return PC_ERR_ARG;
    HIPCHK(hipSetDevice(c->device));
    HIPCHK(hipDeviceSynchronize());
    hipEvent_t epoch = nullptr;
    { std::lock_guard<std::mutex> lk(g_epoch_mu); if (c->device < 16) epoch = g_epoch[c->device]; }
    double ms = 0.0;
    for (size_t i = 0; i + 1 < c->ev_used; i += 2) {
        float t = 0.0f;
        HIPCHK(hipEventElapsedTime(&t, c->ev[i], c->ev[i + 1]));
        ms += t;
        if (i / 2 < c->prof_rec.size()) {
            float s0 = 0.0f;
            if (epoch && hipEventElapsedTime(&s0, epoch, c->ev[i]) != hipSuccess) { (void)hipGetLastError(); s0 = 0.0f; }
            c->prof_rec[i / 2].t0_ms = s0;
            c->prof_rec[i / 2].t1_ms = (double)s0 + t;
        }
    }
    if (const char* path = c->profile_in_schedule ? nullptr : std::getenv("PC_PROFILE_CSV")) {
        if (FILE* f = std::fopen(path, "w")) {
            std::fprintf(f, "i,M,N,K,nphase,epi,gflop,us,tflops,alg_mbytes\n");
            for (size_t i = 0; i < c->prof_rec.size(); ++i) {
                const auto& r = c->prof_rec[i];
                const double t = r.t1_ms - r.t0_ms;
                std::fprintf(f, "%zu,%d,%d,%d,%d,%d,%.3f,%.1f,%.2f,%.3f\n", i, r.M, r.N, r.K, r.nphase, r.epi, r.flops / 1e9, t * 1e3, r.flops / (t * 1e-3) / 1e12, r.bytes / 1e6);
            }
            std::fclose(f);
        }
    }
    *n_launches = (int64_t)(c->ev_used / 2); *total_ms = ms; *total_flops = c->prof_flops;
    c->profile = false; c->ev_used = 0;
    return PC_OK;
}

extern "C" int pc_codec_profile_intervals(const pc_codec* c, double* t0_ms, double* t1_ms, double* flops, size_t cap, size_t* n)
// ... 9 lines not shown
```

### progressivecodec_amd/csrc/pc_conv.hip

```cpp
#include <hip/hip_runtime.h>
#include <stdint.h>
#include <algorithm>
#include <atomic>
#include <cstdio>
#include <cstdlib>
#include <cstring>
#include <mutex>
#include <new>
#include <type_traits>
#include <unordered_map>
#include <utility>
#include <vector>

#include "../../include/pc_math.h"
#include "pc_device.h"

typedef float f32x16 __attribute__((ext_vector_type(16)));
typedef float f32x4 __attribute__((ext_vector_type(4)));

namespace {

__device__ __forceinline__ float epilogue_apply(int epi, float v, float a0, float a1)
{
    switch (epi) {
// ... 472 lines not shown
        }
    }
}


__device__ unsigned long long pc_dbg_stamps[8192][16];

typedef uint32_t u32x4 __attribute__((ext_vector_type(4)));
typedef float f32x4 __attribute__((ext_vector_type(4)));

template <int KQ> __device__ __forceinline__ int pc_swz(int r) { return KQ == 16 ? (r & 15) : (KQ == 4 ? ((r >> 2) & 3) : ((r >> 1) & 7)); }

template <int N> __device__ __forceinline__ void pc_wait_vm()
{
    static_assert(N >= 0 && N < 64, "vmcnt is a 6-bit counter");
    asm volatile("s_waitcnt vmcnt(%0)" ::"n"(N) : "memory");
}
template <int NI, int MAXC> __device__ __forceinline__ void pc_wait_chunks(int chunks)
{
    if constexpr (MAXC <= 0) pc_wait_vm<0>();
    else {
        if (chunks >= MAXC) pc_wait_vm<MAXC * NI>();
        else pc_wait_chunks<NI, MAXC - 1>(chunks);
    }
}

struct pc_run { const float* a_base; const float* w_base; int ld, nch, tap, pad; };

template <int BK, int S, int TM, int TN, bool SQ, int DBG = 0>
__global__ __launch_bounds__(256) __attribute__((amdgpu_waves_per_eu(TM * TN == 1 ? (BK == 16 ? 6 : 5) : 1))) void conv_igemm_uni_kernel(const pc_conv_params p)
{
    constexpr int BM = 64 * TM, BN = 64 * TN, KQ = BK / 4;
    constexpr int NTH = 256;
    constexpr int A_PIECES = BM * KQ, B_PIECES = BN * KQ, STAGE = A_PIECES + B_PIECES;
    constexpr int AIN = A_PIECES / NTH, BIN = B_PIECES / NTH, NI = AIN + BIN;
    constexpr int NG = BK / 8;
    constexpr int NSLOT = NG * 4 * TM * TN;
    static_assert(A_PIECES % NTH == 0 && B_PIECES % NTH == 0 && NI <= NSLOT, "tile / thread mismatch");
    static_assert(S >= 2 && (S - 2) * NI < 64, "vmcnt range");
#if defined(__HIP_DEVICE_COMPILE__)
    extern __shared__ float4 smem[];

    const int wave = __builtin_amdgcn_readfirstlane((int)(threadIdx.x >> 6)), lane = threadIdx.x & 63;
    if (p.dbg & 512) {
        switch ((blockIdx.x >> 8) & 3) {
        case 0: __builtin_amdgcn_s_setprio(3); break;
        case 1: __builtin_amdgcn_s_setprio(2); break;
        case 2: __builtin_amdgcn_s_setprio(1); break;
        default: __builtin_amdgcn_s_setprio(0); break;
        }
    }
    unsigned long long tl[4] = {0, 0, 0, 0};
    if (DBG & 64) tl[0] = __builtin_amdgcn_s_memrealtime();
    const int MT = (p.M + BM - 1) / BM, NT = (p.Cout + BN - 1) / BN, NZ = p.ngroup == 2 ? 2 : p.nphase;
    const int mpx = (MT + 7) >> 3;
    const int xcd = blockIdx.x & 7, slot = blockIdx.x >> 3;
    const int m_local = slot / (NT * NZ), nz = slot - m_local * (NT * NZ);
    int m_tile = p.rowperm ? m_local * 8 + xcd : xcd * mpx + m_local;
    int zsel = nz / NT, n_tile = nz - zsel * NT;
    if (p.group_xcd) {
        const int x4 = xcd & 3, per = 2 * mpx;
        const int ml = slot / NT;
        zsel = xcd >> 2; n_tile = slot - ml * NT;
        m_tile = p.rowperm ? ml * 4 + x4 : x4 * per + ml;
    }
    if (m_tile >= MT) return;
    int phase = zsel;
    const float* seg0_ptr = p.seg[0].ptr;
    const float* wbase = p.w;
    const float* bias = p.bias;
    float* outp = p.out;
    if (p.ngroup == 2 && zsel == 1) { seg0_ptr = p.g1_seg0; wbase = p.g1_w; bias = p.g1_bias; outp = p.g1_out; }
    if (p.ngroup == 2) phase = 0;
    const int m0 = m_tile * BM, n0 = n_tile * BN;
    const int T = p.ntap[phase];
    const int HoWo = p.Ho * p.Wo;
    int chunks_per_tap = 0;
    for (int s = 0; s < p.nseg; ++s) chunks_per_tap += (p.seg[s].nch + BK - 1) / BK;
    int Tv = T;
    uint32_t tmask = T >= 32 ? 0xffffffffu : ((1u << T) - 1u);

    constexpr int OOB = (int)0x80000000;
    int a_q[AIN], a_rel[AIN]; uint32_t a_mask[AIN];
    int64_t pix0;
    if (p.rowtab && p.rowperm) {
        __shared__ int s_minpix;
        __shared__ uint32_t s_tmask;
        if (threadIdx.x == 0) { s_minpix = 0x7fffffff; s_tmask = 0u; }
        __syncthreads();
        int pixv[AIN];
        int mn = 0x7fffffff;
        uint32_t orm = 0u;
#pragma unroll
        for (int i = 0; i < AIN; ++i) {
            const int pa = (wave * AIN + i) * 64 + lane;
            const int row = pa / KQ, sl = pa % KQ;
            a_q[i] = sl ^ pc_swz<KQ>(row);
            const int m = m0 + row;
            const bool ok = m < p.M;
            pixv[i] = ok ? p.rowtab[m] : 0x7fffffff;
            a_mask[i] = ok ? (uint32_t)p.rowtab[(size_t)(1 + phase) * p.M + m] : 0u;
            mn = pixv[i] < mn ? pixv[i] : mn;
            orm |= a_mask[i];
        }
        for (int off = 32; off; off >>= 1) { const int o = __shfl_xor(mn, off); mn = o < mn ? o : mn; orm |= (uint32_t)__shfl_xor((int)orm, off); }
        if (lane == 0) { atomicMin(&s_minpix, mn); atomicOr(&s_tmask, orm); }
        __syncthreads();
        pix0 = s_minpix;
        tmask &= s_tmask;
        if (tmask == 0u) tmask = 1u;
        Tv = __popc(tmask);
#pragma unroll
        for (int i = 0; i < AIN; ++i) a_rel[i] = pixv[i] == 0x7fffffff ? 0 : pixv[i] - (int)pix0;
    } else if (p.rowtab) {
        pix0 = p.rowtab[m0];
#pragma unroll
        for (int i = 0; i < AIN; ++i) {
            const int pa = (wave * AIN + i) * 64 + lane;
            const int row = pa / KQ, sl = pa % KQ;
            a_q[i] = sl ^ pc_swz<KQ>(row);
            const int m = m0 + row;
            const bool ok = m < p.M;
            a_rel[i] = ok ? p.rowtab[m] - (int)pix0 : 0;
            a_mask[i] = ok ? (uint32_t)p.rowtab[(size_t)(1 + phase) * p.M + m] : 0u;
        }
    } else if (p.ident_rows) {
// ... 8 lines not shown
        }
    } else {
        {
            const int b = m0 / HoWo, r = m0 - b * HoWo;
            const int oy = r / p.Wo, ox = r - oy * p.Wo;
            pix0 = ((int64_t)b * p.H + (int64_t)oy * p.stride) * p.W + (int64_t)ox * p.stride;
        }
#pragma unroll
        for (int i = 0; i < AIN; ++i) {
            const int pa = (wave * AIN + i) * 64 + lane;
            const int row = pa / KQ, sl = pa % KQ;
            a_q[i] = sl ^ pc_swz<KQ>(row);
            const int m = m0 + row;
            const bool ok = m < p.M;
            const int mm = ok ? m : m0;
            const int b = mm / HoWo, r = mm - b * HoWo;
            const int oy = r / p.Wo, ox = r - oy * p.Wo;
            const int iy0 = oy * p.stride, ix0 = ox * p.stride;
            a_rel[i] = (int)((((int64_t)b * p.H + iy0) * p.W + ix0) - pix0);
            uint32_t mask = 0;
            for (int t = 0; t < T; ++t) {
                const int iy = iy0 + p.dy[phase][t], ix = ix0 + p.dx[phase][t];
                if ((unsigned)iy < (unsigned)p.H && (unsigned)ix < (unsigned)p.W) mask |= 1u << t;
            }
            a_mask[i] = ok ? mask : 0u;
        }
    }
    int b_q[BIN], b_off[BIN];
#pragma unroll
    for (int i = 0; i < BIN; ++i) {
        const int pb = (wave * BIN + i) * 64 + lane;
        const int row = pb / KQ, sl = pb % KQ;
        b_q[i] = sl ^ pc_swz<KQ>(row);
        b_off[i] = (n0 + row < p.Cout) ? (row * p.Cin + 4 * b_q[i]) * 4 : OOB;
    }
    pc_run* runs = reinterpret_cast<pc_run*>(smem + S * STAGE);
    int runs_per_tap = 0;
    for (int sg = 0; sg < p.nseg; ++sg) runs_per_tap += (p.seg[sg].nch >= BK ? 1 : 0) + (p.seg[sg].nch % BK ? 1 : 0);
    const int nchunks = Tv * chunks_per_tap;
    const int nruns = Tv * runs_per_tap;
    for (int r = threadIdx.x; r < nruns; r += NTH) {
        const int tv = r / runs_per_tap;
        int t = 0;
        { uint32_t mk = tmask; for (int q = 0; q < tv; ++q) mk &= mk - 1u; t = __ffs((int)mk) - 1; }
        int rr = r - tv * runs_per_tap, sg = 0, cbase = 0, ch0 = 0, nch = 0;
        for (;; ++sg) {
            const int full = p.seg[sg].nch / BK * BK, rem = p.seg[sg].nch - full;
            const int here = (full ? 1 : 0) + (rem ? 1 : 0);
            if (rr < here) { const bool is_rem = full ? rr == 1 : true; ch0 = is_rem ? full : 0; nch = is_rem ? rem : full; break; }
            rr -= here; cbase += p.seg[sg].nch;
        }
        pc_run d;
        d.ld = p.seg[sg].ld; d.nch = nch; d.tap = t; d.pad = 0;
        d.a_base = (sg == 0 ? seg0_ptr : p.seg[sg].ptr) + (int64_t)(p.dy[phase][t] * p.W + p.dx[phase][t]) * d.ld + ch0;
        d.w_base = wbase + (int64_t)p.wtap[phase][t] * p.Cout * p.Cin + cbase + ch0;
        runs[r] = d;
    }
    __syncthreads();
    const uint32_t runs_lds = (uint32_t)(uintptr_t)(__attribute__((address_space(3))) void*)runs;
    auto mk = [](uint64_t a) { return __builtin_amdgcn_make_buffer_rsrc(reinterpret_cast<void*>(a), 0, 0x7fffffff, 0x00020000); };
    __amdgpu_buffer_rsrc_t rsrc_a = mk(0), rsrc_b = mk(0);
    int ea[AIN], eb[BIN];
    int run = 0, c_left = 0, koff = 0;
    if (DBG & 4) {
#pragma unroll
        for (int i = 0; i < BIN; ++i) b_off[i] = OOB;
    }
    auto enter_run = [&](int r) {
        u32x4 lo, hi;
        asm volatile("ds_read_b128 %0, %2\n\tds_read_b128 %1, %2 offset:16\n\ts_waitcnt lgkmcnt(0)"
                     : "=&v"(lo), "=&v"(hi) : "v"(runs_lds + (uint32_t)r * 32u) : "memory");
        const uint64_t pa = ((uint64_t)(uint32_t)__builtin_amdgcn_readfirstlane((int)lo.y) << 32) | (uint32_t)__builtin_amdgcn_readfirstlane((int)lo.x);
        const uint64_t pw = ((uint64_t)(uint32_t)__builtin_amdgcn_readfirstlane((int)lo.w) << 32) | (uint32_t)__builtin_amdgcn_readfirstlane((int)lo.z);
        const int d_ld = __builtin_amdgcn_readfirstlane((int)hi.x), d_nch = __builtin_amdgcn_readfirstlane((int)hi.y);
        const int d_tap = __builtin_amdgcn_readfirstlane((int)hi.z);
        auto uni64 = [](uint64_t v) {
            return ((uint64_t)(uint32_t)__builtin_amdgcn_readfirstlane((int)(uint32_t)(v >> 32)) << 32) | (uint32_t)__builtin_amdgcn_readfirstlane((int)(uint32_t)v);
        };
        rsrc_a = mk(uni64(pa + (uint64_t)(pix0 * d_ld) * 4u));
        rsrc_b = mk(uni64(pw + (uint64_t)((int64_t)n0 * p.Cin) * 4u));
        c_left = d_nch; koff = 0;
#pragma unroll
        for (int i = 0; i < AIN; ++i) ea[i] = (((a_mask[i] >> d_tap) & 1u) && 4 * a_q[i] < d_nch && !(DBG & 4)) ? (a_rel[i] * d_ld + 4 * a_q[i]) * 4 : OOB;
#pragma unroll
        for (int i = 0; i < BIN; ++i) eb[i] = (4 * b_q[i] < d_nch) ? b_off[i] : OOB;
    };
    enter_run(0);
    auto piece = [&](int q, int stage) {
        if (DBG & 2) return;
        float4* base = smem + stage * STAGE;
        if (q < AIN)
            __builtin_amdgcn_raw_ptr_buffer_load_lds(rsrc_a, (__attribute__((address_space(3))) void*)(base + (wave * AIN + q) * 64), 16, ea[q < AIN ? q : 0], koff, 0, 0);
        else
            __builtin_amdgcn_raw_ptr_buffer_load_lds(rsrc_b, (__attribute__((address_space(3))) void*)(base + A_PIECES + (wave * BIN + (q - AIN)) * 64), 16,
                                                     eb[q >= AIN ? q - AIN : 0], koff, 0, 0);
    };
    auto advance = [&]() {
        koff += BK * 4;
        c_left -= BK;
        if (c_left <= 0 && ++run < nruns) enter_run(run);
    };

    const int wm = wave >> 1, wn = wave & 1;
    const int half = lane >> 5, l31 = lane & 31;
    const int am = wm * 32 * TM + l31, bn = wn * 32 * TN + l31;
    const int a_swz = pc_swz<KQ>(am), b_swz = pc_swz<KQ>(bn);
    int nlive = 0;
// ... 140 lines not shown
        };
        int c = 0;
        for (; c + S <= n_main - 1; c += S) {
            auto step = [&](auto st_tag) { chunk(nl_tag, std::true_type{}, st_tag, std::integral_constant<int, 1>{}, 0); advance(); };
            step(std::integral_constant<int, 0>{});
            step(std::integral_constant<int, 1 % S>{});
            if constexpr (S >= 3) step(std::integral_constant<int, 2 % S>{});
            if constexpr (S >= 4) step(std::integral_constant<int, 3 % S>{});
            if constexpr (S >= 5) step(std::integral_constant<int, 4 % S>{});
            if constexpr (S >= 6) step(std::integral_constant<int, 5 % S>{});
        }
        auto rest = [&](auto t_tag) {
            constexpr int t = decltype(t_tag)::value;
            if (c + t < nchunks) run_chunk(std::integral_constant<int, t % S>{}, c + t);
        };
        rest(std::integral_constant<int, 0>{});
        rest(std::integral_constant<int, 1>{});
        rest(std::integral_constant<int, 2>{});
        if constexpr (2 * S - 1 > 3) rest(std::integral_constant<int, 3>{});
        if constexpr (2 * S - 1 > 4) rest(std::integral_constant<int, 4>{});
        if constexpr (2 * S - 1 > 5) rest(std::integral_constant<int, 5>{});
        if constexpr (2 * S - 1 > 6) rest(std::integral_constant<int, 6>{});
        if constexpr (2 * S - 1 > 7) rest(std::integral_constant<int, 7>{});
        if constexpr (2 * S - 1 > 8) rest(std::integral_constant<int, 8>{});
        if constexpr (2 * S - 1 > 9) rest(std::integral_constant<int, 9>{});
        if constexpr (2 * S - 1 > 10) rest(std::integral_constant<int, 10>{});
        static_assert(S <= 6, "stages");
        asm volatile("s_waitcnt lgkmcnt(0)" ::: "memory");
    };
    if (DBG & 64) tl[1] = __builtin_amdgcn_s_memrealtime();
    if (nlive == TN) kloop(std::integral_constant<int, TN>{});
    else if (nlive == 0) kloop(std::integral_constant<int, 0>{});
    else kloop(std::integral_constant<int, 1>{});
    if (DBG & 64) tl[2] = __builtin_amdgcn_s_memrealtime();
    __builtin_amdgcn_s_barrier();
    auto stamp_out = [&]() {
        if (!(DBG & 64) || lane != 0 || blockIdx.x >= 8192 / 4) return;
        asm volatile("s_waitcnt vmcnt(0)" ::: "memory");
        unsigned long long* d = pc_dbg_stamps[blockIdx.x * 4 + wave];
        d[0] = tl[0]; d[1] = tl[1]; d[2] = tl[2]; d[3] = __builtin_amdgcn_s_memrealtime();
        d[4] = (unsigned long long)__builtin_amdgcn_s_getreg(0xF804);
        d[5] = (unsigned long long)__builtin_amdgcn_s_getreg(0xF814);
        d[6] = (unsigned long long)nlive; d[7] = (unsigned long long)blockIdx.x;
    };

    if (nlive == 0) { stamp_out(); return; }
    const bool u0 = epilogue_uses_aux0(p.epi), u1 = epilogue_uses_aux1(p.epi);
    const uint32_t epi_bytes = !p.dense_out ? 0u : (u1 ? 32768u : (u0 ? 16384u : 0u));
    const uint32_t tab_byte0 = (uint32_t)(S * STAGE * 16) > epi_bytes ? (uint32_t)(S * STAGE * 16) : epi_bytes;
    uint32_t* rowtab_lds = reinterpret_cast<uint32_t*>(reinterpret_cast<char*>(smem) + tab_byte0) + wave * 64;
    const uint32_t rowtab_lds_addr = smem_lds + tab_byte0 + (uint32_t)wave * 256u;
    const bool fast = TM * TN == 1 && p.out_sc == 1 && (p.dense_out || !u0) && p.epi != PC_EPI_SE_ADD;
    const int ooy_ph = p.ooy[phase], oox_ph = p.oox[phase];
    const float* const aux0_p = p.aux0; const float* const aux1_p = p.aux1;
    const int ld0_v = p.ld0, ld1_v = p.ld1, epi_v = p.epi;
    const int e_Cout = p.Cout, e_M = p.M, e_dense = p.dense_out, e_perm = p.rowperm, e_ps = p.pixel_shuffle, e_osy = p.osy, e_osx = p.osx, e_Wo = p.Wo,
              e_outH = p.outH, e_outW = p.outW;
    const int64_t e_sx = p.out_sx, e_sy = p.out_sy, e_sb = p.out_sb, e_sc = p.out_sc;
    const int* const e_rowtab = p.rowtab;
    float* const e_relu = p.out_relu;
    auto slow_tile = [&](auto i_tag, auto j_tag) __attribute__((always_inline)) {
        constexpr int i = decltype(i_tag)::value, j = decltype(j_tag)::value;
        const int mb = m0 + wm * 32 * TM + i * 32, nb = n0 + (wn * TN + j) * 32;
        const int n = nb + l31;
        const float bv = (bias && n < e_Cout) ? bias[n] : 0.0f;
        for (int r = 0; r < 16; ++r) {
            const int row = (r & 3) + 8 * (r >> 2) + 4 * half;
            const int m = mb + row;
            if (m >= e_M || n >= e_Cout) continue;
            int64_t opix;
            float v = acc[i][j][r];
            if (bias) v = v + bv;
            if (e_dense) {
                opix = e_perm ? (int64_t)e_rowtab[m] : (int64_t)m;
                const float a1 = epi_v == PC_EPI_SE_ADD ? aux1_p[(opix / HoWo) * ld1_v + n] : (u1 ? aux1_p[opix * ld1_v + n] : 0.0f);
                v = epilogue_apply(epi_v, v, u0 ? aux0_p[opix * ld0_v + n] : 0.0f, a1);
                outp[opix * e_sx + (int64_t)n * e_sc] = v;
                if (e_relu) e_relu[opix * e_sx + (int64_t)n * e_sc] = v > 0.0f ? v : 0.0f;
                continue;
            }
            const int b = m / HoWo, rr = m - b * HoWo;
            const int oy = rr / e_Wo, ox = rr - oy * e_Wo;
            const int Y = oy * e_osy + ooy_ph, X = ox * e_osx + oox_ph;
            int nn = n, YY = Y, XX = X;
            if (e_ps) { nn = n >> 2; YY = 2 * Y + ((n >> 1) & 1); XX = 2 * X + (n & 1); }
            const int64_t pix = ((int64_t)b * e_outH + YY) * e_outW + XX;
            v = epilogue_apply(epi_v, v, u0 ? aux0_p[pix * ld0_v + nn] : 0.0f,
                               epi_v == PC_EPI_SE_ADD ? aux1_p[(int64_t)b * ld1_v + nn] : (u1 ? aux1_p[pix * ld1_v + nn] : 0.0f));
            outp[(int64_t)b * e_sb + (int64_t)YY * e_sy + (int64_t)XX * e_sx + (int64_t)nn * e_sc] = v;
        }
    };
    auto fast_tile = [&](auto epi_tag, auto direct_tag, auto i_tag, auto j_tag) __attribute__((always_inline)) {
        constexpr int EPI = decltype(epi_tag)::value, i = decltype(i_tag)::value, j = decltype(j_tag)::value;
        constexpr bool DIRECT = decltype(direct_tag)::value;
        constexpr bool U0 = EPI == PC_EPI_RES_GELU || EPI == PC_EPI_RES || EPI == PC_EPI_GATE || EPI == PC_EPI_GDN || EPI == PC_EPI_IGDN || EPI == PC_EPI_LRP ||
                            EPI == PC_EPI_LRP_ADD || EPI == PC_EPI_LEAKY_RES;
        constexpr bool U1 = EPI == PC_EPI_GATE || EPI == PC_EPI_LRP_ADD;
        float* tile = reinterpret_cast<float*>(smem) + wave * (U1 ? 2048 : 1024);
        const int mb = m0 + wm * 32 * TM + i * 32, nb = n0 + (wn * TN + j) * 32;
        const int n = nb + l31;
        const float bv = (bias && n < e_Cout) ? bias[n] : 0.0f;
        int64_t off0 = 0;
        if (DIRECT) off0 = (int64_t)mb * e_sx;
        else {
            const int m = mb + l31;
            const bool ok = m < e_M;
            int64_t off;
// ... 364 lines not shown
            host[(size_t)p.M + m] = (int)(order[(size_t)m].first == 0u ? full : order[(size_t)m].first);
        }
        if (hipMemcpy(e.tab, host.data(), bytes, hipMemcpyHostToDevice) != hipSuccess) { (void)hipFree(e.tab); (void)hipEventDestroy(e.ready); return nullptr; }
        e.done = true;
    } else {
        hipLaunchKernelGGL(conv_rowtab_kernel, dim3(std::min(2048, (p.M + 255) / 256)), dim3(256), 0, stream, p, e.tab);
        if (hipGetLastError() != hipSuccess || hipEventRecord(e.ready, stream) != hipSuccess) { (void)hipFree(e.tab); (void)hipEventDestroy(e.ready); return nullptr; }
    }
    const int* other = nullptr;
    {
        std::lock_guard<std::mutex> lk(rc->mu);
        if (!(lookup(&other) && other)) {
            e.tick = ++rc->tick;
            rc->bytes += bytes;
            rc->map.emplace(h, e);
            return e.tab;
        }
    }
    std::vector<pc_rowtab_cache::Entry> mine{e};
    pc_rowtab_cache::free_victims(mine);
    return other;
}

void conv_rowtab_unpin(const pc_conv_params& p)
{
    if (!p.rowtab) return;
    pc_rowtab_cache* rc = p.rowtab_cache ? reinterpret_cast<pc_rowtab_cache*>(p.rowtab_cache) : default_rowtab_cache();
    rc->unpin(p.rowtab);
}

template <int BK, int S, int TM, int TN, bool SQ = false, int DBG = 0>
hipError_t launch_uni(const pc_conv_params& p, hipStream_t stream, int* plan)
{
    constexpr int BM = 64 * TM, BN = 64 * TN;
    int tmax = 0;
    for (int ph = 0; ph < p.nphase; ++ph) tmax = std::max(tmax, p.ntap[ph]);
    const bool u1 = p.epi == PC_EPI_GATE || p.epi == PC_EPI_LRP_ADD;
    const bool u0 = u1 || p.epi == PC_EPI_RES_GELU || p.epi == PC_EPI_RES || p.epi == PC_EPI_GDN || p.epi == PC_EPI_IGDN || p.epi == PC_EPI_LRP ||
                    p.epi == PC_EPI_LEAKY_RES || p.epi == PC_EPI_SE_ADD;
    const size_t stage_bytes = (size_t)S * (BM + BN) * (BK / 4) * 16, epi_bytes = !p.dense_out ? 0 : (u1 ? 32768 : (u0 ? 16384 : 0));
    if (plan) {
        plan[0] = (DBG != 0) ? PC_PLAN_UNI_OTHER
                : (SQ && BK == 32 && S == 2 && TM == 1 && TN == 1) ? PC_PLAN_UNI_32_2_SQ
                : (SQ || TM != 1 || TN != 1) ? PC_PLAN_UNI_OTHER
                : (BK == 16 && S == 3) ? PC_PLAN_UNI_16_3 : (BK == 32 && S == 2) ? PC_PLAN_UNI_32_2 : (BK == 32 && S == 3) ? PC_PLAN_UNI_32_3
                : PC_PLAN_UNI_OTHER;
        const bool nchw_ps = TM * TN == 1 && p.pixel_shuffle && !p.dense_out && !u0 && p.out_sx == 1 && p.osx == 1 && p.osy == 1 && p.Wo % 32 == 0 &&
                             p.M % 32 == 0 && (p.Cout & 3) == 0 && stage_bytes >= (size_t)4 * 1056 * 4;
        const bool fast = TM * TN == 1 && p.out_sc == 1 && (p.dense_out || !u0) && p.epi != PC_EPI_SE_ADD;
        const bool direct = p.dense_out && !p.rowperm && (int64_t)32 * p.out_sx * 4 < ((int64_t)1 << 31);
        plan[1] = nchw_ps ? PC_FORM_NCHW_PS : (!fast ? PC_FORM_SLOW : (direct ? PC_FORM_DIRECT : PC_FORM_TABLE));
    }
    const size_t lds = std::max(stage_bytes, epi_bytes) + std::max((size_t)tmax * p.nseg * 2 * sizeof(pc_run), (size_t)1024);
    const int MT = (p.M + BM - 1) / BM, NT = (p.Cout + BN - 1) / BN, NZ = p.ngroup == 2 ? 2 : p.nphase;
    dim3 grid(8 * ((MT + 7) / 8) * NT * NZ, 1, 1);
    auto kern = conv_igemm_uni_kernel<BK, S, TM, TN, SQ, DBG>;
    static std::atomic<uint32_t> attr_set{0};
    int dev = 0;
    (void)hipGetDevice(&dev);
    if (lds > 48 * 1024 && !(attr_set.load(std::memory_order_acquire) & (1u << (dev & 31)))) {
        if (hipFuncSetAttribute(reinterpret_cast<const void*>(kern), hipFuncAttributeMaxDynamicSharedMemorySize, 160 * 1024 - 256) != hipSuccess)
            return hipGetLastError();
        attr_set.fetch_or(1u << (dev & 31), std::memory_order_release);
    }
    static std::atomic<int> printed{0};
    if ((p.dbg & 256) && printed.fetch_add(1) == 0) {
        int nb = -1;
        (void)hipOccupancyMaxActiveBlocksPerMultiprocessor(&nb, kern, 256, lds);
        fprintf(stderr, "[pc_conv] uni<%d,%d,%d,%d> grid %u, lds %zu B, max active blocks per CU %d\n", BK, S, TM, TN, grid.x, lds, nb);
    }
    hipLaunchKernelGGL(kern, grid, dim3(256), lds, stream, p);
    return hipGetLastError();
}

template <int BM, int BN, int WAVES_M, int WAVES_N, bool SMALLC>
hipError_t launch_cfg(const pc_conv_params& p, hipStream_t stream, int* plan)
{
    if (plan) {
        plan[0] = BM == 64 ? (SMALLC ? PC_PLAN_L0_64x64_SMALLC : PC_PLAN_L0_64x64)
                : BN == 32 ? (SMALLC ? PC_PLAN_L0_128x32_SMALLC : PC_PLAN_L0_128x32) : (SMALLC ? PC_PLAN_L0_128x128_SMALLC : PC_PLAN_L0_128x128);
        const bool u0 = p.epi == PC_EPI_RES_GELU || p.epi == PC_EPI_RES || p.epi == PC_EPI_GATE || p.epi == PC_EPI_GDN || p.epi == PC_EPI_IGDN ||
                        p.epi == PC_EPI_LRP || p.epi == PC_EPI_LRP_ADD || p.epi == PC_EPI_LEAKY_RES || p.epi == PC_EPI_SE_ADD;
        plan[1] = (p.dense_out && p.out_sc == 1 && !u0 && (int64_t)32 * p.out_sx * 4 < ((int64_t)1 << 31)) ? PC_FORM_L0_DIRECT : PC_FORM_L0_GENERIC;
    }
    dim3 grid((p.M + BM - 1) / BM, (p.Cout + BN - 1) / BN, p.nphase);
    hipLaunchKernelGGL((conv_igemm_kernel<BM, BN, WAVES_M, WAVES_N, SMALLC>), grid, dim3(256), 0, stream, p);
    return hipGetLastError();
}

}

extern "C" __attribute__((visibility("default"))) int pc_debug_read_stamps(unsigned long long* dst, int nblocks)
{
    if (!dst || nblocks <= 0 || nblocks > 8192) return PC_ERR_ARG;
    return hipMemcpyFromSymbol(dst, HIP_SYMBOL(pc_dbg_stamps), sizeof(unsigned long long) * 16 * (size_t)nblocks) == hipSuccess ? PC_OK : PC_ERR_HIP;
}

int pc_conv_weight_layout(int kind, int Cin, int Cout, int k)
{
    const long ktot = (long)(kind == 0 ? k * k : 9) * Cin;
    return (Cin % 16 == 0 && Cout > 4 && ktot >= 64) ? 1 : 0;
}

int pc_conv_launch(const pc_conv_params& p_in, hipStream_t stream, int* plan)
{
    pc_conv_params p = p_in;
    p.rowtab = nullptr;
    struct Unpin { const pc_conv_params& q; ~Unpin() { conv_rowtab_unpin(q); } } unpin_guard{p};
    if (p.nphase < 1 || p.nphase > 4 || p.M <= 0 || p.Cout <= 0 || p.Cin <= 0) return PC_ERR_ARG;
    static const int dbg_env = (int)pc_tune("PC_CONV_DBG", 0);
    if (dbg_env) p.dbg = dbg_env;
    {
        int tmax = 0;
        for (int ph = 0; ph < p.nphase; ++ph) tmax = std::max(tmax, p.ntap[ph]);
        static const bool no_tab = pc_tune("PC_CONV_NO_ROWTAB", 0) != 0;
        static const bool perm_on = pc_tune("PC_CONV_ROWPERM", 1) != 0;
        static const bool uni_on = pc_tune("PC_CONV_KERN", 1) == 1;
        static const long perm_min_blocks = pc_tune("PC_CONV_ROWPERM_MIN", 256L);
        int maxld = 0;
        for (int sg = 0; sg < p.nseg; ++sg) maxld = std::max(maxld, p.seg[sg].ld);
        maxld = std::max(maxld, std::max(p.ld0, p.ld1));
        maxld = std::max(maxld, (int)std::min<int64_t>(p.out_sx, 0x7fffffff));
        const bool dense = p.nphase == 1 && p.osy == 1 && p.osx == 1 && p.ooy[0] == 0 && p.oox[0] == 0 && p.outH == p.Ho && p.outW == p.Wo &&
                           !p.pixel_shuffle && p.out_sy == (int64_t)p.outW * p.out_sx && p.out_sb == (int64_t)p.outH * p.out_sy;
        p.rowperm = (perm_on && uni_on && !no_tab && p.wlayout == 1 && !p.square && !p.smallc && tmax > 1 && tmax <= 25 && p.nphase == 1 && p.stride == 1 &&
                     p.Ho == p.H && p.Wo == p.W && p.H <= 32 && p.W <= 32 && dense && !(p.dbg & 64) &&
                     (long)((p.M + 63) / 64) * ((p.Cout + 63) / 64) * (p.ngroup == 2 ? 2 : 1) > perm_min_blocks &&
                     (int64_t)p.B * p.H * p.W * (int64_t)std::max(maxld, 1) * 4 < ((int64_t)1 << 31)) ? 1 : 0;
        p.rowtab = (p.wlayout == 1 && tmax > 1 && !no_tab) ? conv_rowtab(p, stream) : nullptr;
        if (!p.rowtab) p.rowperm = 0;
    }
    static const bool group_xcd_on = pc_tune("PC_CONV_GROUP_XCD", 1) != 0;
    p.group_xcd = (group_xcd_on && p.ngroup == 2 && p.wlayout == 1) ? 1 : 0;
    p.ident_rows = p.nphase == 1 && p.ntap[0] == 1 && p.dy[0][0] == 0 && p.dx[0][0] == 0 && p.stride == 1 &&
                                                p.Ho == p.H && p.Wo == p.W;
    p.dense_out = p.nphase == 1 && p.osy == 1 && p.osx == 1 && p.ooy[0] == 0 && p.oox[0] == 0 && p.outH == p.Ho &&
                                               p.outW == p.Wo && !p.pixel_shuffle && p.out_sy == (int64_t)p.outW * p.out_sx &&
                                               p.out_sb == (int64_t)p.outH * p.out_sy;
    if (!p.smallc) {
        int c = 0;
        if (p.nseg < 1 || p.nseg > PC_MAX_SEG) return PC_ERR_ARG;
        for (int s = 0; s < p.nseg; ++s) {
            if (p.seg[s].nch <= 0 || p.seg[s].nch % 16 || p.seg[s].ld % 4 || ((uintptr_t)p.seg[s].ptr & 15)) return PC_ERR_ARG;
            c += p.seg[s].nch;
        }
        if (c != p.Cin) return PC_ERR_ARG;
        if (p.Cout % 4 && p.Cout > 4) return PC_ERR_ARG;
    } else if (p.nseg != 1) return PC_ERR_ARG;
    for (int ph = 0; ph < p.nphase; ++ph)
        if (p.ntap[ph] < 1 || p.ntap[ph] > PC_MAX_TAP) return PC_ERR_ARG;
    if (p.pixel_shuffle && (p.Cout % 4)) return PC_ERR_ARG;
    if (p.epi == PC_EPI_SE_ADD && (!p.aux0 || !p.aux1 || p.nphase != 1)) return PC_ERR_ARG;
    if (p.out_relu && (!p.dense_out || p.out_sc != 1 || p.wlayout != 1 || p.ngroup == 2)) return PC_ERR_ARG;

    hipError_t e;
    if (p.fg_gamma) {
        if (!p.smallc || p.wlayout != 0 || p.Cout != 192 || p.nphase != 1 || !p.dense_out || p.out_sc != 1 || !p.fg_beta || p.epi != PC_EPI_NONE ||
            p.ngroup == 2 || p.ntap[0] * p.Cin > 80)
            return PC_ERR_ARG;
        constexpr size_t lds = (size_t)(64 * 196 + 2 * 192 * 16 + 2 * 80) * sizeof(float);
        if ((int64_t)3 * p.H * p.W >= ((int64_t)1 << 31)) return PC_ERR_ARG;
        static std::atomic<uint32_t> attr_set{0};
        int dev = 0;
        (void)hipGetDevice(&dev);
        if (!(attr_set.load(std::memory_order_acquire) & (1u << (dev & 31)))) {
            if (hipFuncSetAttribute(reinterpret_cast<const void*>(conv_igemm_in_gdn_kernel), hipFuncAttributeMaxDynamicSharedMemorySize, (int)lds) != hipSuccess)
                return PC_ERR_HIP;
            attr_set.fetch_or(1u << (dev & 31), std::memory_order_release);
        }
        if (plan) { plan[0] = PC_PLAN_IN_GDN; plan[1] = PC_FORM_IN_GDN; }
        hipLaunchKernelGGL(conv_igemm_in_gdn_kernel, dim3((unsigned)((p.M + 63) / 64)), dim3(256), lds, stream, p);
        return hipGetLastError() == hipSuccess ? PC_OK : PC_ERR_HIP;
    }
    if (p.wlayout == 1) {
        if (p.smallc || (p.Cin % 16)) return PC_ERR_ARG;
        if (p.ngroup == 2 && (p.nphase != 1 || !p.g1_seg0 || !p.g1_w || !p.g1_out)) return PC_ERR_ARG;
        static const int bk_env = (int)pc_tune("PC_CONV_BK", 0);
        static const int s_env = (int)pc_tune("PC_CONV_S", 0);
        int chunks = 0;
        for (int ph = 0; ph < p.nphase; ++ph) {
            int c = 0;
            for (int sg = 0; sg < p.nseg; ++sg) c += (p.seg[sg].nch + 31) / 32;
            chunks = std::max(chunks, c * p.ntap[ph]);
        }
        const int bk = bk_env ? bk_env : 32;
        const int S = s_env ? s_env : (chunks <= 8 ? 2 : 3);
        static const int kern_env = (int)pc_tune("PC_CONV_KERN", 1);
        static const int tm_env = (int)pc_tune("PC_CONV_TM", 0);
        static const int tn_env = (int)pc_tune("PC_CONV_TN", 0);
        e = hipErrorInvalidValue;
        if (kern_env == 1) {
            const long nb64 = (long)((p.M + 63) / 64) * ((p.Cout + 63) / 64) * (p.ngroup == 2 ? 2 : p.nphase);
            static const int policy = (int)pc_tune("PC_CONV_POLICY", 3);
            static const long small_thr = pc_tune("PC_CONV_SMALL_THR", 256L);
            static const long tm_thr = pc_tune("PC_CONV_TM_THR", 1536L);
            int tm = tm_env ? tm_env : (nb64 >= tm_thr ? 2 : 1), tn = tn_env ? tn_env : 1;
            const int Su = s_env ? s_env : ((chunks <= 8 || tm * tn > 1) ? 2 : 3);
            const int ab = (p.dbg & 64) ? 0 : (p.dbg & 15);
            if (p.square) e = launch_uni<32, 2, 1, 1, true>(p, stream, plan);
#ifdef PC_CONV_TUNING
            else if (ab == 1) e = launch_uni<32, 3, 1, 1, false, 1>(p, stream, plan);
            else if (ab == 2) e = launch_uni<32, 3, 1, 1, false, 2>(p, stream, plan);
            else if (ab == 4) e = launch_uni<32, 3, 1, 1, false, 4>(p, stream, plan);
            else if (ab == 8) e = launch_uni<32, 3, 1, 1, false, 8>(p, stream, plan);
            else if (ab == 10) e = launch_uni<32, 3, 1, 1, false, 10>(p, stream, plan);
            else if (ab == 3) e = launch_uni<32, 3, 1, 1, false, 3>(p, stream, plan);
            else if (ab == 0 && (p.dbg & 16) && !(p.dbg & 64)) e = launch_uni<32, 3, 1, 1, false, 16>(p, stream, plan);
            else if ((p.dbg & 64) && (p.dbg & 8)) e = launch_uni<32, 3, 1, 1, false, 74>(p, stream, plan);
#endif
            else if ((p.dbg & 64) && bk == 16) e = launch_uni<16, 3, 1, 1, false, 64>(p, stream, plan);
            else if (p.dbg & 64) e = launch_uni<32, 3, 1, 1, false, 64>(p, stream, plan);
            else if (bk == 16 && tm == 1 && tn == 1 && s_env == 2) e = launch_uni<16, 2, 1, 1>(p, stream, plan);
            else if (bk == 16 && tm == 1 && tn == 1 && s_env == 3) e = launch_uni<16, 3, 1, 1>(p, stream, plan);
            else if (bk == 16 && tm == 1 && tn == 1) e = launch_uni<16, 4, 1, 1>(p, stream, plan);
            else if (policy == 1 && !s_env && !tm_env && !tn_env) e = launch_uni<16, 3, 1, 1>(p, stream, plan);
            else if (policy == 2 && !s_env && !tm_env && !tn_env && tm == 1) e = launch_uni<16, 3, 1, 1>(p, stream, plan);
            else if (policy == 3 && !s_env && !tm_env && !tn_env && nb64 > small_thr) e = launch_uni<16, 3, 1, 1>(p, stream, plan);
            else if (policy == 3 && !s_env && !tm_env && !tn_env) e = chunks <= 8 ? launch_uni<32, 2, 1, 1>(p, stream, plan) : launch_uni<32, 3, 1, 1>(p, stream, plan);
#define PC_UNI_CASE(S_, TM_, TN_) else if (Su == S_ && tm == TM_ && tn == TN_) e = launch_uni<32, S_, TM_, TN_>(p, stream, plan);
            PC_UNI_CASE(3, 1, 1) PC_UNI_CASE(2, 1, 1) PC_UNI_CASE(3, 2, 1) PC_UNI_CASE(2, 2, 1) PC_UNI_CASE(2, 1, 2)
            PC_UNI_CASE(2, 2, 2)
#undef PC_UNI_CASE
        }
        if (e == hipErrorInvalidValue) return PC_ERR_ARG;
    } else {
        if (p.ngroup == 2) return PC_ERR_ARG;
        int cfg = p.tile_cfg;
        if (cfg == PC_TILE_AUTO) cfg = (p.Cout <= 4) ? PC_TILE_128x32 : PC_TILE_64x64;
        switch (cfg) {
        case PC_TILE_128x128: e = p.smallc ? launch_cfg<128, 128, 2, 2, true>(p, stream, plan) : launch_cfg<128, 128, 2, 2, false>(p, stream, plan); break;
        case PC_TILE_64x64: e = p.smallc ? launch_cfg<64, 64, 2, 2, true>(p, stream, plan) : launch_cfg<64, 64, 2, 2, false>(p, stream, plan); break;
        case PC_TILE_128x32: e = p.smallc ? launch_cfg<128, 32, 4, 1, true>(p, stream, plan) : launch_cfg<128, 32, 4, 1, false>(p, stream, plan); break;
        default: return PC_ERR_ARG;
        }
    }
    return e == hipSuccess ? PC_OK : PC_ERR_HIP;
}
```

### progressivecodec_amd/csrc/pc_device.h

```cpp
#ifndef PC_DEVICE_H
#define PC_DEVICE_H

#include <hip/hip_runtime.h>
#include <stdint.h>

#include "../../include/pcodec.h"

#ifdef PC_TUNING
#include <cstdlib>
static inline long pc_tune(const char* name, long dflt) { const char* v = std::getenv(name); return v ? std::atol(v) : dflt; }
#else
static inline constexpr long pc_tune(const char*, long dflt) { return dflt; }
#endif

#define PC_MAX_SEG 8
#define PC_MAX_TAP 25

enum {
    PC_EPI_NONE = 0,
    PC_EPI_GELU = 1,
    PC_EPI_RES_GELU = 2,
    PC_EPI_RES = 3,
    PC_EPI_GATE = 4,
    PC_EPI_GDN = 5,
    PC_EPI_IGDN = 6,
    PC_EPI_CLAMP01 = 7,
    PC_EPI_LRP = 8,
    PC_EPI_LRP_ADD = 9,
    PC_EPI_LEAKY = 10,
    PC_EPI_LEAKY_RES = 11,
    PC_EPI_RELU = 12,
    PC_EPI_SE_ADD = 13,
};

enum { PC_TILE_AUTO = 0, PC_TILE_128x128 = 1, PC_TILE_64x64 = 2, PC_TILE_128x32 = 3 };

struct pc_seg {
    const float* ptr;
    int ld;
    int nch;
};

struct pc_conv_params {
    pc_seg seg[PC_MAX_SEG];
    int nseg, Cin;
    int B, H, W;
    int smallc;
    int64_t in_sb, in_sy, in_sx, in_sc;
    int square;
    int nphase;
    int ntap[4];
    int dy[4][PC_MAX_TAP], dx[4][PC_MAX_TAP];
    int wtap[4][PC_MAX_TAP];
    int stride;
    const float* w;
    int wlayout;
    const float* bias;
    int Cout;
    int Ho, Wo, M;
    int osy, osx, ooy[4], oox[4];
    int outH, outW;
    int64_t out_sb, out_sy, out_sx, out_sc;
    float* out;
    int pixel_shuffle;
    float* out_relu;
    int epi;
    const float* aux0; int ld0;
    const float* aux1; int ld1;
    int tile_cfg;
    const float* fg_gamma; const float* fg_beta;
    int ngroup;
    const float* g1_seg0; const float* g1_w; const float* g1_bias; float* g1_out;
    const int* rowtab;
    void* rowtab_cache;
    int ident_rows;
    int dense_out;
    int rowperm;
    int group_xcd;
    int dbg;
};

int pc_conv_launch(const pc_conv_params& p, hipStream_t stream, int* plan = nullptr);
struct pc_rowtab_cache;
pc_rowtab_cache* pc_rowtab_cache_create(size_t cap_bytes);
void pc_rowtab_cache_destroy(pc_rowtab_cache* c);
size_t pc_rowtab_cache_bytes(pc_rowtab_cache* c);
int pc_conv_weight_layout(int kind, int Cin, int Cout, int k);

int pc_win_attention_launch(const float* qkv, const float* bias, int B, int H, int W, int C, int heads, int ws,
                            int shift, float scale, float* out, hipStream_t stream, int bias_ji = 0, int* plan = nullptr);

struct pc_prep_params {
    int B, HW, C;
    const float* scale; int ld_scale;
    const float* mu; int ld_mu;
    const float* y; int ld_y;
    const float* ybase; int ld_ybase;
    const float* thr;
    const float* mask_src; int64_t mask_sb;
    int mask_mode;
    const float* table; int ntable; float bound;
    int32_t* sym;
    int32_t* idx;
    uint8_t* idx8;
    float* mask;
    float* yhat; int ld_yhat;
    const float* yadd; int ld_yadd;
    float* lik; int64_t lik_sb;
};
int pc_prep_enc_launch(const pc_prep_params& p, hipStream_t stream, int* plan = nullptr);
int pc_prep_dec_index_launch(const pc_prep_params& p, hipStream_t stream, int* plan = nullptr);
int pc_prep_dec_dequant_launch(const pc_prep_params& p, hipStream_t stream, int* plan = nullptr);

int pc_quantile_thr_launch(const float* scale, int ld, int B, int HW, int C, float q, float* thr, uint32_t* work,
                           hipStream_t stream, int64_t batch_stride = 0, int* plan = nullptr);
size_t pc_quantile_work_bytes(int B);
#define PC_QUANTILE_SMALL_N 32768

int pc_rem_combine_launch(const float* ret, int ld_ret, float* scale, int ld_scale, int B, int HW, const float* thr_star, int mode_star,
                          const float* thr_bar, int mode_bar, hipStream_t stream, float* mu = nullptr, int ld_mu = 0);
#define PC_SE_CHUNK 4096
int pc_se_squeeze_launch(const float* x, int B, int HW, int C, const float* fc1, const float* fc2, float* part, float* s, hipStream_t stream);
int pc_maxpool2_launch(const float* x, int B, int H, int W, int C, float* out, hipStream_t stream);
int pc_nchw_slice_to_nhwc_launch(const float* src, int64_t batch_stride, int B, int HW, int C, float* dst, hipStream_t stream);

// ... 10 lines not shown
```

### progressivecodec_amd/csrc/pc_host.cpp

```cpp
#include <pthread.h>
#include <sched.h>

#include <algorithm>
#include <atomic>
#include <cmath>
#include <cstdio>
#include <condition_variable>
#include <cstdlib>
#include <cstring>
#include <functional>
#include <mutex>
#include <thread>
#include <vector>

#include "../../include/pc_math.h"
#include "../../include/pcodec.h"
#include "pc_host.h"

namespace {
constexpr uint64_t kRansL = 1ull << 31;
constexpr int kPrecision = 16;
constexpr int kBypassBits = 4;
constexpr int kBypassMax = 15;

struct Writer {
    uint32_t* begin;
    uint32_t* ptr;
    bool overflow = false;
    inline void put(uint32_t w) { if (ptr == begin) { overflow = true; return; } *--ptr = w; }
};

inline void enc_put(uint64_t& x, Writer& wr, uint32_t start, uint32_t freq)
{
    const uint64_t x_max = ((kRansL >> kPrecision) << 32) * freq;
    if (x >= x_max) { wr.put((uint32_t)x); x >>= 32; }
    x = ((x / freq) << kPrecision) + (x % freq) + start;
}
inline void enc_put_bits(uint64_t& x, Writer& wr, uint32_t val)
{
    const uint32_t freq = 1u << (16 - kBypassBits);
    const uint64_t x_max = ((kRansL >> 16) << 32) * freq;
    if (x >= x_max) { wr.put((uint32_t)x); x >>= 32; }
    x = (x << kBypassBits) | val;
}
}

extern "C" size_t pc_rans_bound(size_t n)
{
    return 4 * (3 * n + 4);
}

extern "C" int pc_rans_encode_with_indexes(const int32_t* symbols, const int32_t* indexes, size_t n,
                                           const int32_t* cdfs, int n_cdf, int cdf_stride,
                                           const int32_t* cdf_sizes, const int32_t* offsets,
                                           uint8_t* out, size_t out_cap, size_t* out_len)
{
    if ((!symbols || !indexes) && n) return PC_ERR_ARG;
    if (!cdfs || !cdf_sizes || !offsets || !out || !out_len || n_cdf <= 0 || cdf_stride <= 0) return PC_ERR_ARG;
    const size_t cap_words = out_cap / 4;
    if (cap_words < 2) return PC_ERR_BUFFER;
    uint32_t* base = reinterpret_cast<uint32_t*>(out);
    if (reinterpret_cast<uintptr_t>(out) & 3) return PC_ERR_ARG;
    Writer wr{base, base + cap_words};
    uint64_t x = kRansL;
    for (size_t ii = n; ii-- > 0;) {
        const int32_t ci = indexes[ii];
        if (ci < 0 || ci >= n_cdf) return PC_ERR_INDEX;
        const int32_t len = cdf_sizes[ci];
        if (len < 2 || len > cdf_stride) return PC_ERR_CDF;
        const int32_t* cdf = cdfs + (size_t)ci * cdf_stride;
// ... 410 lines not shown
                                    const int32_t* cdfs, int n_cdf, int cdf_stride,
                                    const int32_t* cdf_sizes, const int32_t* offsets,
                                    uint8_t* out, size_t out_stride, size_t* out_lens, int n_threads)
{
    if (!out || !out_lens || (out_stride & 3) || ((!symbols || !indexes) && n && n_streams)) return PC_ERR_ARG;
    std::atomic<int> rc{PC_OK};
    auto job = [&](size_t s) {
        const int r = pc_rans_encode_with_indexes(symbols + s * n, indexes + s * n, n, cdfs, n_cdf, cdf_stride, cdf_sizes,
                                                  offsets, out + s * out_stride, out_stride, &out_lens[s]);
        if (r != PC_OK) rc = r;
    };
    if (n_threads == 1) for (size_t s = 0; s < n_streams; ++s) job(s);
    else pc::default_pool().parallel_for(n_streams, job);
    return rc;
}

extern "C" int pc_rans_decode_batch(const uint8_t* const* encoded, const size_t* encoded_lens, size_t n_streams,
                                    const int32_t* indexes, size_t n,
                                    const int32_t* cdfs, int n_cdf, int cdf_stride,
                                    const int32_t* cdf_sizes, const int32_t* offsets,
                                    int32_t* out, int n_threads)
{
    if (!encoded || !encoded_lens || ((!indexes || !out) && n && n_streams)) return PC_ERR_ARG;
    for (size_t s = 0; s < n_streams; ++s) if (!encoded[s]) return PC_ERR_ARG;
    std::atomic<int> rc{PC_OK};
    auto job = [&](size_t s) {
        const int r = pc_rans_decode_with_indexes(encoded[s], encoded_lens[s], indexes + s * n, n, cdfs, n_cdf, cdf_stride,
                                                  cdf_sizes, offsets, out + s * n);
        if (r != PC_OK) rc = r;
    };
    if (n_threads == 1) for (size_t s = 0; s < n_streams; ++s) job(s);
    else pc::default_pool().parallel_for(n_streams, job);
    return rc;
}

extern "C" int pc_rans_decode_batch_u8(const uint8_t* const* encoded, const size_t* encoded_lens, size_t n_streams,
                                       const uint8_t* indexes, size_t n,
                                       const int32_t* cdfs, int n_cdf, int cdf_stride,
                                       const int32_t* cdf_sizes, const int32_t* offsets,
                                       int32_t* out, int n_threads)
{
    if (!cdfs || !cdf_sizes || !offsets || n_cdf <= 0 || n_cdf > 256 || cdf_stride < 2) return PC_ERR_ARG;
    for (int i = 0; i < n_cdf; ++i) {
        const int32_t* row = cdfs + (size_t)i * cdf_stride;
        if (cdf_sizes[i] < 2 || cdf_sizes[i] > cdf_stride || row[0] != 0 || row[cdf_sizes[i] - 1] != (1 << 16)) return PC_ERR_CDF;
        for (int j = 0; j + 1 < cdf_sizes[i]; ++j) if (row[j + 1] <= row[j]) return PC_ERR_CDF;
    }
    std::vector<uint64_t> lut((size_t)n_cdf * 256);
    pc::build_decode_lut(cdfs, n_cdf, cdf_stride, cdf_sizes, lut.data());
    return pc::rans_decode_u8_batch(encoded, encoded_lens, n_streams, indexes, n, pc::DecTables{cdfs, n_cdf, cdf_stride, cdf_sizes, offsets, lut.data()}, out,
                                    n_threads);
}

extern "C" const char* pc_version(void) { return "progressivecodec_amd 0.3 (gfx950), numeric contract 0x00020001"; }
extern "C" uint32_t pc_contract_id(void) { return PC_NUMERIC_CONTRACT_ID; }

extern "C" const char* pc_strerror(int code)
{
    switch (code) {
    case PC_OK: return "ok";
    case PC_ERR_ARG: return "invalid argument or unsupported shape";
    case PC_ERR_INDEX: return "CDF index out of range";
    case PC_ERR_BUFFER: return "output buffer too small";
    case PC_ERR_TRUNCATED: return "truncated bitstream";
    case PC_ERR_CDF: return "malformed CDF / pmf";
    case PC_ERR_HIP: return "HIP runtime error";
    case PC_ERR_NOMEM: return "out of memory";
    case PC_ERR_STATE: return "object not ready (tables or weights missing; run update()/finalize first)";
    case PC_ERR_MISSING: return "state_dict tensor missing or of the wrong shape";
    default: return "unknown error";
    }
}
```

Baseline: 48.07.

## Batch independent base-slice context stacks into one grouped conv launch

Generalizes the conv kernel's two-group mode to up to ten groups, each with its own weights, inputs, outputs and aux pointers, mapped onto XCDs through a shared tile-map helper. The channel-model chain then runs the last base slices' mean/scale stacks and LRP stacks as one grouped launch per layer instead of one slice at a time. The goal is fewer small kernel launches and better GPU occupancy on small latent grids. In exchange the per-group workspace grows, the parameter struct gets much larger, and the slice dependency order and host buffer offsets change.

```diff
diff --git a/include/pcodec.h b/include/pcodec.h
--- a/include/pcodec.h
+++ b/include/pcodec.h
@@ -213,6 +213,15 @@
 #define PC_FORM_L0_GENERIC 6
 #define PC_FORM_IN_GDN 7
 PC_API int pc_test_conv(const pc_test_conv_desc* d, int* plan, void* stream);
+typedef struct pc_test_conv_group {
+    const float* seg_ptr[PC_TEST_MAX_SEG];
+    const float* w; const float* bias;
+    float* out;
+    const float* aux0; const float* aux1;
+} pc_test_conv_group;
+PC_API int pc_test_conv_groups(const pc_test_conv_desc* d, const pc_test_conv_group* groups, int G, int* plan, void* stream);
+PC_API int pc_conv_tile_map(int block, int MT, int NT, int G, int rowperm, int* group, int* m_tile, int* n_tile);
+PC_API int pc_conv_tile_grid(int MT, int NT, int G);
 
 typedef struct pc_test_stage_desc {
     int size;
diff --git a/progressivecodec_amd/_lib.py b/progressivecodec_amd/_lib.py
--- a/progressivecodec_amd/_lib.py
+++ b/progressivecodec_amd/_lib.py
@@ -22,6 +22,7 @@
     "pc_codec_set_post_filter", "pc_codec_post_filter",
     "pc_codec_set_model", "pc_codec_wacnn_compress", "pc_codec_wacnn_decompress", "pc_codec_wacnn_forward",
     "pc_test_conv", "pc_codec_set_topology", "pc_test_stage",
+    "pc_test_conv_groups", "pc_conv_tile_map", "pc_conv_tile_grid",
 ]
 
 
@@ -81,6 +82,8 @@
             L.pc_selftest_packed_gelu.argtypes = [C.POINTER(C.c_uint64), C.POINTER(C.c_uint64)]
         if hasattr(L, "pc_test_conv"):
             L.pc_test_conv.argtypes = [vp, C.POINTER(C.c_int), vp]
+        if hasattr(L, "pc_test_conv_groups"):
+            L.pc_test_conv_groups.argtypes = [vp, vp, C.c_int, C.POINTER(C.c_int), vp]
         if hasattr(L, "pc_test_stage"):
             L.pc_test_stage.argtypes = [vp, C.POINTER(C.c_int), vp]
         L.pc_codec_compress.argtypes = [vp, vp, C.c_int, C.c_int, C.c_int, C.c_double, C.c_int, vp, vp]
diff --git a/progressivecodec_amd/csrc/pc_codec.hip b/progressivecodec_amd/csrc/pc_codec.hip
--- a/progressivecodec_amd/csrc/pc_codec.hip
+++ b/progressivecodec_amd/csrc/pc_codec.hip
@@ -120,6 +120,7 @@
     hipEvent_t eFork = nullptr;
     std::mutex buf_mu;
     double t_host_decode_ms = 0.0;
+    int n_base_handovers = 0;
     double t_compress_ms = 0.0, t_host_encode_ms = 0.0, t_host_encode_exposed_ms = 0.0, t_decompress_ms = 0.0;
     double n_sym_encoded = 0.0, n_sym_decoded = 0.0;
     int last_B = 0, last_h16 = 0, last_w16 = 0;
@@ -161,16 +162,24 @@
     if (!c) return pc_conv_launch(q, st, plan);
     long taps = 0;
     for (int ph = 0; ph < q.nphase; ++ph) taps += q.ntap[ph];
-    const double ng = q.ngroup == 2 ? 2.0 : 1.0;
+    const double ng = q.ngroup ? (double)q.ngroup : 1.0;
     double fl = 2.0 * (double)q.M * (double)q.Cout * (double)taps * (double)q.Cin * ng;
     if (q.fg_gamma) fl += 2.0 * (double)q.M * (double)q.Cout * (double)q.Cout;
     double by = 0.0;
-    for (int sg = 0; sg < q.nseg; ++sg) by += 4.0 * (double)q.B * q.H * q.W * q.seg[sg].nch * (sg == 0 ? ng : 1.0);
+    for (int sg = 0; sg < q.nseg; ++sg) {
+        int distinct = 1;
+        for (int g = 1; g < q.ngroup; ++g) {
+            bool seen = q.grp[g].seg[sg] == q.seg[sg].ptr;
+            for (int g2 = 1; g2 < g && !seen; ++g2) seen = q.grp[g2].seg[sg] == q.grp[g].seg[sg];
+            distinct += seen ? 0 : 1;
+        }
+        by += 4.0 * (double)q.B * q.H * q.W * q.seg[sg].nch * distinct;
+    }
     by += ng * 4.0 * ((double)taps * q.Cin * q.Cout + q.Cout);
     if (q.fg_gamma) by += 4.0 * ((double)q.Cout * q.Cout + q.Cout);
     by += ng * 4.0 * (double)q.nphase * q.M * q.Cout;
-    if (q.aux0 && q.epi != PC_EPI_NONE && q.epi != PC_EPI_GELU && q.epi != PC_EPI_CLAMP01) by += 4.0 * (double)q.nphase * q.M * q.Cout;
-    if (q.aux1 && (q.epi == PC_EPI_GATE || q.epi == PC_EPI_LRP_ADD)) by += 4.0 * (double)q.nphase * q.M * q.Cout;
+    if (q.aux0 && q.epi != PC_EPI_NONE && q.epi != PC_EPI_GELU && q.epi != PC_EPI_CLAMP01) by += ng * 4.0 * (double)q.nphase * q.M * q.Cout;
+    if (q.aux1 && (q.epi == PC_EPI_GATE || q.epi == PC_EPI_LRP_ADD)) by += ng * 4.0 * (double)q.nphase * q.M * q.Cout;
     hipEvent_t e0, e1;
     {
         std::lock_guard<std::mutex> lk(c->prof_mu);
@@ -465,7 +474,10 @@
     q.out_sc = 1; q.out_sx = ldo; q.out_sy = (int64_t)q.outW * ldo; q.out_sb = (int64_t)q.outH * q.outW * ldo;
     if (g1) {
         if (g1->w->Cin != w.Cin || g1->w->Cout != w.Cout || g1->w->k != w.k || g1->w->layout != 1 || w.layout != 1) return PC_ERR_ARG;
-        q.ngroup = 2; q.g1_seg0 = g1->seg0; q.g1_w = g1->w->w; q.g1_bias = g1->w->b; q.g1_out = g1->out;
+        q.ngroup = 2;
+        pc_conv_group& e = q.grp[1];
+        for (int j = 0; j < q.nseg; ++j) e.seg[j] = q.seg[j].ptr;
+        e.seg[0] = g1->seg0; e.w = g1->w->w; e.bias = g1->w->b; e.out = g1->out; e.aux0 = aux0; e.aux1 = aux1;
     }
     return launch_conv(q, st);
 }
@@ -576,6 +588,71 @@
     return stack5_pair_n(c, st, sm, ss, segs_mean.begin(), (int)segs_mean.size(), seg0_scale, B, h, w, out_mean, out_scale, tagm, tags);
 }
 
+struct StackGroup { const Stack5W* s; const float* in[PC_MAX_SEG]; float* out; const float* aux0; };
+
+int conv_groups(hipStream_t st, const ConvW* const* ws, const Seg* segs, int nseg, const float* const (*ins)[PC_MAX_SEG], int G, int B, int H, int W,
+                float* const* outs, int ldo, int epi, const float* const* aux0s, int ld0)
+{
+    if (G < 1 || G > PC_MAX_GROUP || nseg < 1 || nseg > PC_MAX_SEG) return PC_ERR_ARG;
+    pc_conv_params q;
+    std::memset(&q, 0, sizeof(q));
+    const ConvW& w = *ws[0];
+    int cin = 0;
+    for (int j = 0; j < nseg; ++j) {
+        if (segs[j].nch <= 0) return PC_ERR_ARG;
+        q.seg[j].ptr = ins[0][j]; q.seg[j].ld = segs[j].ld; q.seg[j].nch = segs[j].nch; cin += segs[j].nch;
+    }
+    q.nseg = nseg;
+    if (cin != w.Cin || w.layout != 1) return PC_ERR_ARG;
+    q.Cin = cin;
+    q.w = w.w; q.wlayout = w.layout; q.bias = w.b; q.Cout = w.Cout;
+    q.epi = epi; q.aux0 = aux0s ? aux0s[0] : nullptr; q.ld0 = ld0;
+    q.out = outs[0];
+    PCCHK(conv_geometry(q, w.kind == 0 ? 0 : 1, w.k, 1, H, W, B, false));
+    q.out_sc = 1; q.out_sx = ldo; q.out_sy = (int64_t)q.outW * ldo; q.out_sb = (int64_t)q.outH * q.outW * ldo;
+    q.ngroup = G;
+    for (int g = 1; g < G; ++g) {
+        const ConvW& wg = *ws[g];
+        if (wg.Cin != w.Cin || wg.Cout != w.Cout || wg.k != w.k || wg.kind != w.kind || wg.layout != 1 || (wg.b == nullptr) != (w.b == nullptr)) return PC_ERR_ARG;
+        pc_conv_group& e = q.grp[g];
+        for (int j = 0; j < nseg; ++j) e.seg[j] = ins[g][j];
+        e.w = wg.w; e.bias = wg.b; e.out = outs[g]; e.aux0 = aux0s ? aux0s[g] : nullptr; e.aux1 = nullptr;
+    }
+    return launch_conv(q, st);
+}
+
+int stack5_groups(pc_codec* c, hipStream_t st, const StackGroup* sg, int G, const Seg* segs, int nseg, int B, int h, int w, int ldo, int epi, int ld0,
+                  const std::string& tag)
+{
+    if (G < 1 || G > PC_MAX_GROUP) return PC_ERR_ARG;
+    const size_t M = (size_t)B * h * w;
+    float *t0[PC_MAX_GROUP], *t1[PC_MAX_GROUP], *outs[PC_MAX_GROUP];
+    const float* aux0s[PC_MAX_GROUP];
+    const ConvW* ws[PC_MAX_GROUP];
+    const float* ins[PC_MAX_GROUP][PC_MAX_SEG];
+    for (int g = 0; g < G; ++g) {
+        PCCHK(c->buf(tag + "_" + std::to_string(g) + "_t0", M * 224, &t0[g]));
+        PCCHK(c->buf(tag + "_" + std::to_string(g) + "_t1", M * 176, &t1[g]));
+    }
+    auto layer = [&](int l, const Seg* sgs, int ns, float* const* o, int ld_o, int e, const float* const* a0, int ld_a0) {
+        for (int g = 0; g < G; ++g) ws[g] = &sg[g].s->c[l];
+        return conv_groups(st, ws, sgs, ns, ins, G, B, h, w, o, ld_o, e, a0, ld_a0);
+    };
+    for (int g = 0; g < G; ++g) for (int j = 0; j < nseg; ++j) ins[g][j] = sg[g].in[j];
+    PCCHK(layer(0, segs, nseg, t0, 224, PC_EPI_GELU, nullptr, 0));
+    const int width[3] = {224, 176, 128}, next[3] = {176, 128, 64};
+    for (int l = 1; l <= 3; ++l) {
+        float* const* src = (l & 1) ? t0 : t1;
+        float* const* dst = (l & 1) ? t1 : t0;
+        for (int g = 0; g < G; ++g) ins[g][0] = src[g];
+        const Seg one{nullptr, width[l - 1], width[l - 1]};
+        PCCHK(layer(l, &one, 1, dst, next[l - 1], PC_EPI_GELU, nullptr, 0));
+    }
+    for (int g = 0; g < G; ++g) { ins[g][0] = t1[g]; outs[g] = sg[g].out; aux0s[g] = sg[g].aux0; }
+    const Seg last{nullptr, 64, 64};
+    return layer(4, &last, 1, outs, ldo, epi, epi == PC_EPI_NONE ? nullptr : aux0s, ld0);
+}
+
 int hs(pc_codec* c, hipStream_t st, const HsW& h, const float* z, int B, int zh, int zw, float* out, int ldo)
 {
     const size_t M = (size_t)B * zh * zw;
@@ -882,7 +959,41 @@
     else q.wlayout = d->kind == 1 ? pc_conv_weight_layout(1, d->Cin, d->Cout, 5) : 1;
     q.out = d->out; q.out_sb = d->out_sb; q.out_sy = d->out_sy; q.out_sx = d->out_sx; q.out_sc = d->out_sc;
     q.out_relu = d->out_relu;
-    if (d->ngroup == 2) { q.ngroup = 2; q.g1_seg0 = d->g1_seg0; q.g1_w = d->g1_w; q.g1_bias = d->g1_bias; q.g1_out = d->g1_out; }
+    if (d->ngroup == 2) {
+        q.ngroup = 2;
+        pc_conv_group& e = q.grp[1];
+        for (int s = 0; s < d->nseg; ++s) e.seg[s] = d->seg_ptr[s];
+        e.seg[0] = d->g1_seg0; e.w = d->g1_w; e.bias = d->g1_bias; e.out = d->g1_out; e.aux0 = d->aux0; e.aux1 = d->aux1;
+    }
+    return pc_conv_launch(q, (hipStream_t)stream, plan);
+}
+
+extern "C" int pc_test_conv_groups(const pc_test_conv_desc* d, const pc_test_conv_group* groups, int G, int* plan, void* stream)
+{
+    if (plan) plan[0] = plan[1] = 0;
+    if (!d || !groups || G < 1 || G > PC_MAX_GROUP || d->ngroup != 0) return PC_ERR_ARG;
+    if (d->nseg < 1 || d->nseg > PC_MAX_SEG || d->B <= 0 || d->H <= 0 || d->W <= 0) return PC_ERR_ARG;
+    if (d->smallc || d->fg_gamma || d->out_relu) return PC_ERR_ARG;
+    pc_conv_params q;
+    std::memset(&q, 0, sizeof(q));
+    q.nseg = d->nseg;
+    for (int s = 0; s < d->nseg; ++s) { q.seg[s].ptr = groups[0].seg_ptr[s]; q.seg[s].ld = d->seg_ld[s]; q.seg[s].nch = d->seg_nch[s]; }
+    q.Cin = d->Cin;
+    q.square = d->square ? 1 : 0;
+    q.w = groups[0].w; q.bias = groups[0].bias; q.Cout = d->Cout; q.tile_cfg = d->tile_cfg;
+    q.epi = d->epi; q.aux0 = groups[0].aux0; q.ld0 = d->ld0; q.aux1 = groups[0].aux1; q.ld1 = d->ld1;
+    if (d->kind == 2 && d->Cout != 12) return PC_ERR_ARG;
+    PCCHK(conv_geometry(q, d->kind, d->k, d->stride, d->H, d->W, d->B, d->pixel_shuffle != 0));
+    if (d->kind == 0) q.wlayout = q.square ? 1 : pc_conv_weight_layout(0, d->Cin, d->Cout, d->k);
+    else q.wlayout = d->kind == 1 ? pc_conv_weight_layout(1, d->Cin, d->Cout, 5) : 1;
+    q.out = groups[0].out; q.out_sb = d->out_sb; q.out_sy = d->out_sy; q.out_sx = d->out_sx; q.out_sc = d->out_sc;
+    q.ngroup = G;
+    for (int g = 1; g < G; ++g) {
+        pc_conv_group& e = q.grp[g];
+        for (int s = 0; s < d->nseg; ++s) e.seg[s] = groups[g].seg_ptr[s];
+        e.w = groups[g].w; e.bias = groups[g].bias; e.out = groups[g].out; e.aux0 = groups[g].aux0; e.aux1 = groups[g].aux1;
+    }
+    if (!q.out || !q.w) return PC_ERR_ARG;
     return pc_conv_launch(q, (hipStream_t)stream, plan);
 }
 
@@ -1597,13 +1708,21 @@
     return conv(st, c->joiner[i][2], {{jb, 64, 64}}, nb, k.h, k.w, 1, ye, D0, PC_EPI_NONE);
 }
 
-int chain_workspace(pc_codec* c, const std::string& tag, size_t m)
+constexpr int WIDE0 = 5, NWIDE = NS0 - WIDE0;
+bool wide_base(const ChainCtx& k, int step) { return k.c->model == PC_MODEL_CHANNEL && !k.sig && step == WIDE0 && k.step1 >= NS0; }
+
+int chain_workspace(pc_codec* c, const std::string& tag, size_t m, bool wide)
 {
     float* d;
     for (const char* base : {"s5m", "s5s"}) {
         PCCHK(c->buf(base + tag + "_t0", m * 224, &d));
         PCCHK(c->buf(base + tag + "_t1", m * 176, &d));
     }
+    if (wide && c->model == PC_MODEL_CHANNEL)
+        for (int g = 0; g < 2 * NWIDE; ++g) {
+            PCCHK(c->buf("s5w" + tag + "_" + std::to_string(g) + "_t0", m * 224, &d));
+            PCCHK(c->buf("s5w" + tag + "_" + std::to_string(g) + "_t1", m * 176, &d));
+        }
     if (!c->topo.joiner_cond) return PC_OK;
     PCCHK(c->buf("jn_pm" + tag, m * SLICE, &d));
     PCCHK(c->buf("jn_a" + tag, m * 64, &d));
@@ -1693,23 +1812,69 @@
     return joiner(k, i, b0, nb, pm, sA, tag);
 }
 
+int wide_params(const ChainCtx& k, int b0, int nb, hipStream_t st, const std::string& tag)
+{
+    pc_codec* c = k.c;
+    const size_t pi = (size_t)k.HW;
+    const float* lm = img(k.lm, b0, pi * MLAT); const float* ls = img(k.ls, b0, pi * MLAT);
+    const float* yb = img(k.yb, b0, pi * D0);
+    StackGroup sg[2 * NWIDE];
+    std::memset(sg, 0, sizeof(sg));
+    for (int j = 0; j < NWIDE; ++j) {
+        const int i = WIDE0 + j;
+        sg[j].s = &c->cc_mean[i]; sg[j].in[0] = lm; sg[j].in[1] = yb; sg[j].out = k.mu + slice_off(k, i, b0);
+        sg[NWIDE + j].s = &c->cc_scale[i]; sg[NWIDE + j].in[0] = ls; sg[NWIDE + j].in[1] = yb; sg[NWIDE + j].out = k.scale + slice_off(k, i, b0);
+    }
+    const Seg segs[2] = {{nullptr, MLAT, D0}, {nullptr, D0, 32 * 5}};
+    return stack5_groups(c, st, sg, 2 * NWIDE, segs, 2, nb, k.h, k.w, SLICE, PC_EPI_NONE, 0, "s5w" + tag);
+}
+
+int wide_lrp(const ChainCtx& k, int b0, int nb, hipStream_t st, const std::string& tag)
+{
+    pc_codec* c = k.c;
+    const size_t pi = (size_t)k.HW;
+    const float* lm = img(k.lm, b0, pi * MLAT);
+    float* yb = img(k.yb, b0, pi * D0);
+    StackGroup sg[NWIDE];
+    std::memset(sg, 0, sizeof(sg));
+    for (int j = 0; j < NWIDE; ++j) {
+        const int i = WIDE0 + j;
+        sg[j].s = &c->lrp[i]; sg[j].in[0] = lm; sg[j].in[1] = yb; sg[j].in[2] = yb + 32 * i; sg[j].out = yb + 32 * i; sg[j].aux0 = yb + 32 * i;
+    }
+    const Seg segs[3] = {{nullptr, MLAT, D0}, {nullptr, D0, 160}, {nullptr, D0, 32}};
+    return stack5_groups(c, st, sg, NWIDE, segs, 3, nb, k.h, k.w, D0, PC_EPI_LRP, D0, "s5w" + tag);
+}
+
 int encode_lane(const ChainCtx& k, int b0, int nb, hipStream_t sA, const std::string& tag)
 {
     pc_codec* c = k.c;
     const size_t pi = (size_t)k.HW;
     for (int step = k.step0; step < k.step1; ++step) {
-        PCCHK(chain_wait(k, step, sA));
-        PCCHK(chain_params(k, step, b0, nb, sA, tag));
-        const size_t so = slice_off(k, step, b0);
-        pc_prep_params p = chain_prep(k, step, b0, nb);
-        p.mu = k.mu + so; p.ld_mu = SLICE; p.y = img(k.y, b0, pi * MLAT) + 32 * step; p.ld_y = MLAT;
-        p.sym = k.sym + so;
-        p.lik = k.lik ? k.lik + ((size_t)b0 * k.lik_nch + (size_t)32 * step) * pi : nullptr;
-        p.lik_sb = (int64_t)k.lik_nch * (int64_t)pi;
-        if (step < NS0) {
-            p.yhat = img(k.yb, b0, pi * D0) + 32 * step; p.ld_yhat = D0;
-            PCCHK(pc_prep_enc_launch(p, sA));
-        } else {
+        const bool wide = wide_base(k, step);
+        const int nstep = wide ? NWIDE : 1;
+        for (int s2 = step; s2 < step + nstep; ++s2) PCCHK(chain_wait(k, s2, sA));
+        if (wide) PCCHK(wide_params(k, b0, nb, sA, tag));
+        else PCCHK(chain_params(k, step, b0, nb, sA, tag));
+        pc_prep_params p;
+        for (int s2 = step; s2 < step + nstep; ++s2) {
+            const size_t so = slice_off(k, s2, b0);
+            p = chain_prep(k, s2, b0, nb);
+            p.mu = k.mu + so; p.ld_mu = SLICE; p.y = img(k.y, b0, pi * MLAT) + 32 * s2; p.ld_y = MLAT;
+            p.sym = k.sym + so;
+            p.lik = k.lik ? k.lik + ((size_t)b0 * k.lik_nch + (size_t)32 * s2) * pi : nullptr;
+            p.lik_sb = (int64_t)k.lik_nch * (int64_t)pi;
+            if (s2 < NS0) {
+                p.yhat = img(k.yb, b0, pi * D0) + 32 * s2; p.ld_yhat = D0;
+                PCCHK(pc_prep_enc_launch(p, sA));
+            }
+        }
+        if (wide) {
+            PCCHK(wide_lrp(k, b0, nb, sA, tag));
+            for (int s2 = step; s2 < step + nstep; ++s2) PCCHK(chain_signal(k, s2, sA));
+            step += nstep - 1;
+            continue;
+        }
+        if (step >= NS0) {
             const int i = step - NS0;
             const pc_topology& T = c->topo;
             p.mask = k.masks ? k.masks + slice_off(k, i, b0) : nullptr;
@@ -1736,29 +1901,54 @@
     HIPCHK(hipSetDevice(c->device));
     LaunchState launch(c);
     const size_t pi = (size_t)k.HW, per = (size_t)SLICE * k.HW;
-    int32_t* h_idx = c->h_idx + k.h_off + (size_t)b0 * per;
-    int32_t* h_sym = c->h_sym + k.h_off + (size_t)b0 * per;
+    const bool base = k.step0 < NS0;
+    const size_t hw = base ? (size_t)NWIDE : 1;
+    int32_t* h_idx = c->h_idx + k.h_off + hw * (size_t)b0 * per;
+    int32_t* h_sym = c->h_sym + k.h_off + hw * (size_t)b0 * per;
+    uint8_t* h_idx8 = reinterpret_cast<uint8_t*>(h_idx);
+    std::vector<const uint8_t*> w_str;
+    std::vector<size_t> w_len;
     for (int step = k.step0; step < k.step1; ++step) {
-        PCCHK(chain_wait(k, step, sA));
-        PCCHK(chain_params(k, step, b0, nb, sA, tag));
-        const size_t so = slice_off(k, step, b0);
+        const bool wide = wide_base(k, step);
+        const int nstep = wide ? NWIDE : 1;
+        for (int j = 0; j < nstep; ++j) PCCHK(chain_wait(k, step + j, sA));
+        if (wide) PCCHK(wide_params(k, b0, nb, sA, tag));
+        else PCCHK(chain_params(k, step, b0, nb, sA, tag));
         const bool e = step >= NS0;
         const int i = e ? step - NS0 : step;
-        pc_prep_params p = chain_prep(k, step, b0, nb);
-        p.idx8 = k.idx8 + so;
-        PCCHK(pc_prep_dec_index_launch(p, sA));
-        uint8_t* h_idx8 = reinterpret_cast<uint8_t*>(h_idx);
-        HIPCHK(hipMemcpyAsync(h_idx8, k.idx8 + so, per * nb, hipMemcpyDeviceToHost, sA));
+        for (int j = 0; j < nstep; ++j) {
+            const size_t so = slice_off(k, step + j, b0);
+            pc_prep_params p = chain_prep(k, step + j, b0, nb);
+            p.idx8 = k.idx8 + so;
+            PCCHK(pc_prep_dec_index_launch(p, sA));
+            HIPCHK(hipMemcpyAsync(h_idx8 + (size_t)j * nb * per, k.idx8 + so, per * nb, hipMemcpyDeviceToHost, sA));
+        }
         HIPCHK(hipStreamSynchronize(sA));
         const double td0 = now_ms();
         const size_t slot = e ? (size_t)NS0 + (size_t)NS0 * k.level + i : (size_t)step;
-        PCCHK(pc::rans_decode_u8_batch(y_strings + slot * k.B + b0, y_lens + slot * k.B + b0, nb, h_idx8, per, c->gc.dec(), h_sym, nt));
-        { std::lock_guard<std::mutex> lk(c->buf_mu); c->t_host_decode_ms += now_ms() - td0; }
-        HIPCHK(hipMemcpyAsync(k.sym + so, h_sym, per * nb * 4, hipMemcpyHostToDevice, sA));
-        float* dst = e ? img(k.ye, b0, pi * D0) + 32 * i : img(k.yb, b0, pi * D0) + 32 * i;
-        PCCHK(pc_gc_dequantize(k.sym + so, k.mu + so, SLICE, nb, k.HW, dst, D0, sA));
-        PCCHK(chain_lrp(k, step, b0, nb, sA, tag));
-        PCCHK(chain_signal(k, step, sA));
+        const uint8_t* const* str = y_strings + slot * k.B + b0;
+        const size_t* len = y_lens + slot * k.B + b0;
+        if (wide) {
+            w_str.resize((size_t)nstep * nb); w_len.resize((size_t)nstep * nb);
+            for (int j = 0; j < nstep; ++j)
+                for (int b = 0; b < nb; ++b) {
+                    w_str[(size_t)j * nb + b] = y_strings[(slot + j) * k.B + b0 + b];
+                    w_len[(size_t)j * nb + b] = y_lens[(slot + j) * k.B + b0 + b];
+                }
+            str = w_str.data(); len = w_len.data();
+        }
+        PCCHK(pc::rans_decode_u8_batch(str, len, (size_t)nstep * nb, h_idx8, per, c->gc.dec(), h_sym, nt));
+        { std::lock_guard<std::mutex> lk(c->buf_mu); c->t_host_decode_ms += now_ms() - td0; if (base) ++c->n_base_handovers; }
+        for (int j = 0; j < nstep; ++j) {
+            const size_t so = slice_off(k, step + j, b0);
+            HIPCHK(hipMemcpyAsync(k.sym + so, h_sym + (size_t)j * nb * per, per * nb * 4, hipMemcpyHostToDevice, sA));
+            float* dst = e ? img(k.ye, b0, pi * D0) + 32 * i : img(k.yb, b0, pi * D0) + 32 * (i + j);
+            PCCHK(pc_gc_dequantize(k.sym + so, k.mu + so, SLICE, nb, k.HW, dst, D0, sA));
+        }
+        if (wide) PCCHK(wide_lrp(k, b0, nb, sA, tag));
+        else PCCHK(chain_lrp(k, step, b0, nb, sA, tag));
+        for (int j = 0; j < nstep; ++j) PCCHK(chain_signal(k, step + j, sA));
+        step += nstep - 1;
     }
     return PC_OK;
 }
@@ -1773,7 +1963,7 @@
     PCCHK(ensure_lanes(c, nl));
     for (int g = 0; g < nl; ++g) {
         const int b0 = (int)((long)k.B * g / nl), nb = (int)((long)k.B * (g + 1) / nl) - b0;
-        PCCHK(chain_workspace(c, std::to_string(g), (size_t)nb * k.HW));
+        PCCHK(chain_workspace(c, std::to_string(g), (size_t)nb * k.HW, k.step0 < NS0));
     }
     HIPCHK(hipEventRecord(c->eFork, st));
     for (int g = 0; g < nl; ++g) HIPCHK(hipStreamWaitEvent(c->lanes[g].sA, c->eFork, 0));
@@ -1855,7 +2045,7 @@
         c->pipe_ev.resize(NS0 + 2);
         for (auto& e : c->pipe_ev) HIPCHK(hipEventCreateWithFlags(&e, hipEventDisableTiming));
     }
-    for (const char* tag : {"PA", "PB"}) PCCHK(chain_workspace(c, tag, M));
+    for (const char* tag : {"PA", "PB"}) PCCHK(chain_workspace(c, tag, M, false));
     return PC_OK;
 }
 
@@ -2008,7 +2198,7 @@
     const size_t per = (size_t)SLICE * k.HW, per_z = (size_t)NCH * k.ZHW;
     if (c->staging_pending) { HIPCHK(hipEventSynchronize(c->staging_done)); c->staging_pending = false; }
     if (!c->staging_done) HIPCHK(hipEventCreateWithFlags(&c->staging_done, hipEventDisableTiming));
-    PCCHK(ensure_host_staging(c, std::max(per * k.B, per_z * k.B)));
+    PCCHK(ensure_host_staging(c, std::max(NWIDE * per * k.B, per_z * k.B)));
     eb_indexes(c->h_idx, per_z * k.B, k.ZHW);
     PCCHK(pc_rans_decode_batch(z_strings, z_lens, k.B, c->h_idx, per_z, c->eb.cdf.data(), c->eb.n, c->eb.stride, c->eb.len.data(),
                                c->eb.off.data(), c->h_sym, c->n_threads == 1 ? 1 : 0));
@@ -2245,17 +2435,18 @@
     PCCHK(decoder_front(k, st, z_strings, z_lens, any_enh));
     const int nt = c->n_threads == 1 ? 1 : 0;
     c->t_host_decode_ms = 0.0;
+    c->n_base_handovers = 0;
     int first_enh = -1;
     for (int l = 0; l < n_levels && first_enh < 0; ++l) if (qualities[l] != 0) first_enh = l;
     const bool piped = pipeline_enabled(c) && first_enh >= 0;
     if (piped) {
         PCCHK(ensure_pipeline(c, M));
-        PCCHK(ensure_host_staging(c, std::max(2 * per * B, per_z * B)));
+        PCCHK(ensure_host_staging(c, std::max((NWIDE + 1) * per * B, per_z * B)));
         SliceSignal recorded;
         ChainCtx kb = k;
         kb.sig = c->pipe_ev.data(); kb.sig_count = &recorded;
         ChainCtx ke = level_ctx(k, first_enh, qualities[first_enh], mask_pol);
-        ke.waitv = c->pipe_ev.data(); ke.wait_count = &recorded; ke.h_off = per * B;
+        ke.waitv = c->pipe_ev.data(); ke.wait_count = &recorded; ke.h_off = NWIDE * per * B;
         PCCHK(decode_pair(kb, ke, st, y_strings, y_lens, nt));
     } else {
         PCCHK(run_chain(k, st, true, y_strings, y_lens));
@@ -2476,6 +2667,7 @@
     if (!c || !out || n < 6) return PC_ERR_ARG;
     out[0] = c->t_compress_ms; out[1] = c->t_host_encode_ms; out[2] = c->t_host_encode_exposed_ms;
     out[3] = c->t_host_decode_ms; out[4] = c->n_sym_encoded; out[5] = c->n_sym_decoded;
+    if (n >= 7) out[6] = (double)c->n_base_handovers;
     return PC_OK;
 }
 
diff --git a/progressivecodec_amd/csrc/pc_conv.hip b/progressivecodec_amd/csrc/pc_conv.hip
--- a/progressivecodec_amd/csrc/pc_conv.hip
+++ b/progressivecodec_amd/csrc/pc_conv.hip
@@ -548,26 +548,27 @@
     }
     unsigned long long tl[4] = {0, 0, 0, 0};
     if (DBG & 64) tl[0] = __builtin_amdgcn_s_memrealtime();
-    const int MT = (p.M + BM - 1) / BM, NT = (p.Cout + BN - 1) / BN, NZ = p.ngroup == 2 ? 2 : p.nphase;
+    const int MT = (p.M + BM - 1) / BM, NT = (p.Cout + BN - 1) / BN, NZ = p.ngroup ? p.ngroup : p.nphase;
     const int mpx = (MT + 7) >> 3;
     const int xcd = blockIdx.x & 7, slot = blockIdx.x >> 3;
     const int m_local = slot / (NT * NZ), nz = slot - m_local * (NT * NZ);
     int m_tile = p.rowperm ? m_local * 8 + xcd : xcd * mpx + m_local;
     int zsel = nz / NT, n_tile = nz - zsel * NT;
     if (p.group_xcd) {
-        const int x4 = xcd & 3, per = 2 * mpx;
-        const int ml = slot / NT;
-        zsel = xcd >> 2; n_tile = slot - ml * NT;
-        m_tile = p.rowperm ? ml * 4 + x4 : x4 * per + ml;
+        if (!pc_tilemap_tile((int)blockIdx.x, MT, NT, p.ngroup, p.rowperm, &zsel, &m_tile, &n_tile)) return;
     }
     if (m_tile >= MT) return;
     int phase = zsel;
-    const float* seg0_ptr = p.seg[0].ptr;
     const float* wbase = p.w;
     const float* bias = p.bias;
     float* outp = p.out;
-    if (p.ngroup == 2 && zsel == 1) { seg0_ptr = p.g1_seg0; wbase = p.g1_w; bias = p.g1_bias; outp = p.g1_out; }
-    if (p.ngroup == 2) phase = 0;
+    const float* aux0_p = p.aux0; const float* aux1_p = p.aux1;
+    const int gsel = p.ngroup ? __builtin_amdgcn_readfirstlane(zsel) : 0;
+    if (p.ngroup) {
+        const pc_conv_group& ge = p.grp[gsel];
+        wbase = ge.w; bias = ge.bias; outp = ge.out; aux0_p = ge.aux0; aux1_p = ge.aux1;
+        phase = 0;
+    }
     const int m0 = m_tile * BM, n0 = n_tile * BN;
     const int T = p.ntap[phase];
     const int HoWo = p.Ho * p.Wo;
@@ -682,7 +683,7 @@
         }
         pc_run d;
         d.ld = p.seg[sg].ld; d.nch = nch; d.tap = t; d.pad = 0;
-        d.a_base = (sg == 0 ? seg0_ptr : p.seg[sg].ptr) + (int64_t)(p.dy[phase][t] * p.W + p.dx[phase][t]) * d.ld + ch0;
+        d.a_base = (p.ngroup ? p.grp[gsel].seg[sg] : p.seg[sg].ptr) +(int64_t)(p.dy[phase][t] * p.W + p.dx[phase][t]) * d.ld + ch0;
         d.w_base = wbase + (int64_t)p.wtap[phase][t] * p.Cout * p.Cin + cbase + ch0;
         runs[r] = d;
     }
@@ -929,7 +930,6 @@
     const uint32_t rowtab_lds_addr = smem_lds + tab_byte0 + (uint32_t)wave * 256u;
     const bool fast = TM * TN == 1 && p.out_sc == 1 && (p.dense_out || !u0) && p.epi != PC_EPI_SE_ADD;
     const int ooy_ph = p.ooy[phase], oox_ph = p.oox[phase];
-    const float* const aux0_p = p.aux0; const float* const aux1_p = p.aux1;
     const int ld0_v = p.ld0, ld1_v = p.ld1, epi_v = p.epi;
     const int e_Cout = p.Cout, e_M = p.M, e_dense = p.dense_out, e_perm = p.rowperm, e_ps = p.pixel_shuffle, e_osy = p.osy, e_osx = p.osx, e_Wo = p.Wo,
               e_outH = p.outH, e_outW = p.outW;
@@ -1400,8 +1400,8 @@
         plan[1] = nchw_ps ? PC_FORM_NCHW_PS : (!fast ? PC_FORM_SLOW : (direct ? PC_FORM_DIRECT : PC_FORM_TABLE));
     }
     const size_t lds = std::max(stage_bytes, epi_bytes) + std::max((size_t)tmax * p.nseg * 2 * sizeof(pc_run), (size_t)1024);
-    const int MT = (p.M + BM - 1) / BM, NT = (p.Cout + BN - 1) / BN, NZ = p.ngroup == 2 ? 2 : p.nphase;
-    dim3 grid(8 * ((MT + 7) / 8) * NT * NZ, 1, 1);
+    const int MT = (p.M + BM - 1) / BM, NT = (p.Cout + BN - 1) / BN, NZ = p.ngroup ? p.ngroup : p.nphase;
+    dim3 grid(p.group_xcd ? pc_tilemap_grid(MT, NT, p.ngroup) : 8 * ((MT + 7) / 8) * NT * NZ, 1, 1);
     auto kern = conv_igemm_uni_kernel<BK, S, TM, TN, SQ, DBG>;
     static std::atomic<uint32_t> attr_set{0};
     int dev = 0;
@@ -1456,6 +1456,12 @@
     p.rowtab = nullptr;
     struct Unpin { const pc_conv_params& q; ~Unpin() { conv_rowtab_unpin(q); } } unpin_guard{p};
     if (p.nphase < 1 || p.nphase > 4 || p.M <= 0 || p.Cout <= 0 || p.Cin <= 0) return PC_ERR_ARG;
+    if (p.ngroup < 0 || p.ngroup > PC_MAX_GROUP) return PC_ERR_ARG;
+    if (p.ngroup) {
+        pc_conv_group& g0 = p.grp[0];
+        for (int sg = 0; sg < PC_MAX_SEG; ++sg) g0.seg[sg] = sg < p.nseg ? p.seg[sg].ptr : nullptr;
+        g0.w = p.w; g0.bias = p.bias; g0.out = p.out; g0.aux0 = p.aux0; g0.aux1 = p.aux1;
+    }
     static const int dbg_env = (int)pc_tune("PC_CONV_DBG", 0);
     if (dbg_env) p.dbg = dbg_env;
     {
@@ -1473,13 +1479,13 @@
                            !p.pixel_shuffle && p.out_sy == (int64_t)p.outW * p.out_sx && p.out_sb == (int64_t)p.outH * p.out_sy;
         p.rowperm = (perm_on && uni_on && !no_tab && p.wlayout == 1 && !p.square && !p.smallc && tmax > 1 && tmax <= 25 && p.nphase == 1 && p.stride == 1 &&
                      p.Ho == p.H && p.Wo == p.W && p.H <= 32 && p.W <= 32 && dense && !(p.dbg & 64) &&
-                     (long)((p.M + 63) / 64) * ((p.Cout + 63) / 64) * (p.ngroup == 2 ? 2 : 1) > perm_min_blocks &&
+                     (long)((p.M + 63) / 64) * ((p.Cout + 63) / 64) * (p.ngroup ? p.ngroup : 1) > perm_min_blocks &&
                      (int64_t)p.B * p.H * p.W * (int64_t)std::max(maxld, 1) * 4 < ((int64_t)1 << 31)) ? 1 : 0;
         p.rowtab = (p.wlayout == 1 && tmax > 1 && !no_tab) ? conv_rowtab(p, stream) : nullptr;
         if (!p.rowtab) p.rowperm = 0;
     }
     static const bool group_xcd_on = pc_tune("PC_CONV_GROUP_XCD", 1) != 0;
-    p.group_xcd = (group_xcd_on && p.ngroup == 2 && p.wlayout == 1) ? 1 : 0;
+    p.group_xcd = (group_xcd_on && p.ngroup && p.wlayout == 1) ? 1 : 0;
     p.ident_rows = p.nphase == 1 && p.ntap[0] == 1 && p.dy[0][0] == 0 && p.dx[0][0] == 0 && p.stride == 1 &&
                                                 p.Ho == p.H && p.Wo == p.W;
     p.dense_out = p.nphase == 1 && p.osy == 1 && p.osx == 1 && p.ooy[0] == 0 && p.oox[0] == 0 && p.outH == p.Ho &&
@@ -1499,12 +1505,12 @@
         if (p.ntap[ph] < 1 || p.ntap[ph] > PC_MAX_TAP) return PC_ERR_ARG;
     if (p.pixel_shuffle && (p.Cout % 4)) return PC_ERR_ARG;
     if (p.epi == PC_EPI_SE_ADD && (!p.aux0 || !p.aux1 || p.nphase != 1)) return PC_ERR_ARG;
-    if (p.out_relu && (!p.dense_out || p.out_sc != 1 || p.wlayout != 1 || p.ngroup == 2)) return PC_ERR_ARG;
+    if (p.out_relu && (!p.dense_out || p.out_sc != 1 || p.wlayout != 1 || p.ngroup)) return PC_ERR_ARG;
 
     hipError_t e;
     if (p.fg_gamma) {
         if (!p.smallc || p.wlayout != 0 || p.Cout != 192 || p.nphase != 1 || !p.dense_out || p.out_sc != 1 || !p.fg_beta || p.epi != PC_EPI_NONE ||
-            p.ngroup == 2 || p.ntap[0] * p.Cin > 80)
+            p.ngroup || p.ntap[0] * p.Cin > 80)
             return PC_ERR_ARG;
         constexpr size_t lds = (size_t)(64 * 196 + 2 * 192 * 16 + 2 * 80) * sizeof(float);
         if ((int64_t)3 * p.H * p.W >= ((int64_t)1 << 31)) return PC_ERR_ARG;
@@ -1522,7 +1528,19 @@
     }
     if (p.wlayout == 1) {
         if (p.smallc || (p.Cin % 16)) return PC_ERR_ARG;
-        if (p.ngroup == 2 && (p.nphase != 1 || !p.g1_seg0 || !p.g1_w || !p.g1_out)) return PC_ERR_ARG;
+        if (p.ngroup) {
+            if (p.nphase != 1) return PC_ERR_ARG;
+            const bool u1 = p.epi == PC_EPI_GATE || p.epi == PC_EPI_LRP_ADD;
+            const bool u0 = u1 || p.epi == PC_EPI_RES_GELU || p.epi == PC_EPI_RES || p.epi == PC_EPI_GDN || p.epi == PC_EPI_IGDN || p.epi == PC_EPI_LRP ||
+                            p.epi == PC_EPI_LEAKY_RES;
+            if (p.epi == PC_EPI_SE_ADD) return PC_ERR_ARG;
+            for (int g = 0; g < p.ngroup; ++g) {
+                const pc_conv_group& ge = p.grp[g];
+                if (!ge.w || !ge.out || (u0 && !ge.aux0) || (u1 && !ge.aux1)) return PC_ERR_ARG;
+                for (int sg = 0; sg < p.nseg; ++sg)
+                    if (!ge.seg[sg] || ((uintptr_t)ge.seg[sg] & 15)) return PC_ERR_ARG;
+            }
+        }
         static const int bk_env = (int)pc_tune("PC_CONV_BK", 0);
         static const int s_env = (int)pc_tune("PC_CONV_S", 0);
         int chunks = 0;
@@ -1538,7 +1556,7 @@
         static const int tn_env = (int)pc_tune("PC_CONV_TN", 0);
         e = hipErrorInvalidValue;
         if (kern_env == 1) {
-            const long nb64 = (long)((p.M + 63) / 64) * ((p.Cout + 63) / 64) * (p.ngroup == 2 ? 2 : p.nphase);
+            const long nb64 = (long)((p.M + 63) / 64) * ((p.Cout + 63) / 64) * (p.ngroup ? p.ngroup : p.nphase);
             static const int policy = (int)pc_tune("PC_CONV_POLICY", 3);
             static const long small_thr = pc_tune("PC_CONV_SMALL_THR", 256L);
             static const long tm_thr = pc_tune("PC_CONV_TM_THR", 1536L);
@@ -1572,7 +1590,7 @@
         }
         if (e == hipErrorInvalidValue) return PC_ERR_ARG;
     } else {
-        if (p.ngroup == 2) return PC_ERR_ARG;
+        if (p.ngroup) return PC_ERR_ARG;
         int cfg = p.tile_cfg;
         if (cfg == PC_TILE_AUTO) cfg = (p.Cout <= 4) ? PC_TILE_128x32 : PC_TILE_64x64;
         switch (cfg) {
diff --git a/progressivecodec_amd/csrc/pc_conv_tilemap.h b/progressivecodec_amd/csrc/pc_conv_tilemap.h
--- /dev/null
+++ b/progressivecodec_amd/csrc/pc_conv_tilemap.h
@@ -0,0 +1,40 @@
+#ifndef PC_CONV_TILEMAP_H
+#define PC_CONV_TILEMAP_H
+
+#if defined(__HIPCC__)
+#define PC_TILEMAP_FN __host__ __device__ static inline
+#else
+#define PC_TILEMAP_FN static inline
+#endif
+
+#define PC_MAX_GROUP 10
+
+PC_TILEMAP_FN int pc_conv_share_begin(int x, int L) { return (int)(((long long)x * L) >> 3); }
+
+PC_TILEMAP_FN int pc_tilemap_grid(int MT, int NT, int G) { return 8 * ((G * MT + 7) >> 3) * NT; }
+
+PC_TILEMAP_FN bool pc_tilemap_tile(int block, int MT, int NT, int G, int rowperm, int* group, int* m_tile, int* n_tile)
+{
+    const int L = G * MT, xcd = block & 7, slot = block >> 3;
+    const int s = pc_conv_share_begin(xcd, L), e = pc_conv_share_begin(xcd + 1, L);
+    const int ml = slot / NT;
+    if (ml >= e - s) return false;
+    const int idx = s + ml, g = idx / MT;
+    *group = g;
+    *n_tile = slot - ml * NT;
+    if (!rowperm) { *m_tile = idx - g * MT; return true; }
+    const int g0 = g * MT, g1 = g0 + MT;
+    const int k = idx - (s > g0 ? s : g0);
+    int m = 0;
+    for (int x = 0; x < 8; ++x) {
+        const int xs = pc_conv_share_begin(x, L), xe = pc_conv_share_begin(x + 1, L);
+        const int c = (xe < g1 ? xe : g1) - (xs > g0 ? xs : g0);
+        if (c <= 0) continue;
+        m += c < k ? c : k;
+        if (x < xcd && c > k) ++m;
+    }
+    *m_tile = m;
+    return true;
+}
+
+#endif
diff --git a/progressivecodec_amd/csrc/pc_device.h b/progressivecodec_amd/csrc/pc_device.h
--- a/progressivecodec_amd/csrc/pc_device.h
+++ b/progressivecodec_amd/csrc/pc_device.h
@@ -5,6 +5,7 @@
 #include <stdint.h>
 
 #include "../../include/pcodec.h"
+#include "pc_conv_tilemap.h"
 
 #ifdef PC_TUNING
 #include <cstdlib>
@@ -41,6 +42,13 @@
     int nch;
 };
 
+struct pc_conv_group {
+    const float* seg[PC_MAX_SEG];
+    const float* w; const float* bias;
+    float* out;
+    const float* aux0; const float* aux1;
+};
+
 struct pc_conv_params {
     pc_seg seg[PC_MAX_SEG];
     int nseg, Cin;
@@ -70,7 +78,7 @@
     int tile_cfg;
     const float* fg_gamma; const float* fg_beta;
     int ngroup;
-    const float* g1_seg0; const float* g1_w; const float* g1_bias; float* g1_out;
+    pc_conv_group grp[PC_MAX_GROUP];
     const int* rowtab;
     void* rowtab_cache;
     int ident_rows;
diff --git a/progressivecodec_amd/csrc/pc_host.cpp b/progressivecodec_amd/csrc/pc_host.cpp
--- a/progressivecodec_amd/csrc/pc_host.cpp
+++ b/progressivecodec_amd/csrc/pc_host.cpp
@@ -16,6 +16,7 @@
 #include "../../include/pc_math.h"
 #include "../../include/pcodec.h"
 #include "pc_host.h"
+#include "pc_conv_tilemap.h"
 
 namespace {
 constexpr uint64_t kRansL = 1ull << 31;
@@ -532,6 +533,13 @@
                                     n_threads);
 }
 
+extern "C" int pc_conv_tile_map(int block, int MT, int NT, int G, int rowperm, int* group, int* m_tile, int* n_tile)
+{
+    if (block < 0 || MT < 1 || NT < 1 || G < 1 || G > PC_MAX_GROUP || !group || !m_tile || !n_tile) return 0;
+    return pc_tilemap_tile(block, MT, NT, G, rowperm ? 1 : 0, group, m_tile, n_tile) ? 1 : 0;
+}
+extern "C" int pc_conv_tile_grid(int MT, int NT, int G) { return (MT < 1 || NT < 1 || G < 1 || G > PC_MAX_GROUP) ? 0 : pc_tilemap_grid(MT, NT, G); }
+
 extern "C" const char* pc_version(void) { return "progressivecodec_amd 0.3 (gfx950), numeric contract 0x00020001"; }
 extern "C" uint32_t pc_contract_id(void) { return PC_NUMERIC_CONTRACT_ID; }
 
```

New measurement: 47.60. 1.0% lower.
